# nmndeep/Robust-Segmentation

Hardware: AMD Instinct MI355X
Metric: SEA attack-iterations/sec (UperNet-CNX-T, 512x512) (higher is better)
Workload: dtype f32 (frozen-weight GEMMs on the 16-bit matrix cores by operand splitting: fp16x2 (22 significant bits per operand, 3 MFMA products) forward, fp16x2 (22 significant bits per operand, 3 MFMA products) input gradient; fp32 storage and accumulate)

## Files before the change

include/sea_hip.h:

```cpp
#ifndef SEA_HIP_H
#define SEA_HIP_H

#include <stddef.h>
#include <stdint.h>

#ifdef __cplusplus
extern "C" {
#endif

#define SEA_MODE_MASK_CE 0
#define SEA_MODE_MASK_CE_BAL 1
#define SEA_MODE_JS 2
#define SEA_MODE_CE 3

#define SEA_DTYPE_F32 0
#define SEA_DTYPE_BF16 1
#define SEA_DTYPE_F16 2

#define SEA_LAYOUT_NCHW 0
#define SEA_LAYOUT_NHWC 1

int sea_abi_version(void);
const char* sea_build_info(void);
int sea_fastdiv_magic(uint32_t d, uint32_t* m, uint32_t* s);
// ... 74 lines not shown
int sea_dwconv7x7_nhwc(const float* x, const float* wt, const float* bias, float* y, int B, int C,
                       int H, int W, int flip, void* stream);
int sea_dwconv7x7_nhwc_add(const float* x, const float* wt, const float* bias, const float* addend, float* y, int B,
                           int C, int H, int W, int flip, void* stream);

int sea_upsample_bilinear_fwd(const float* x, float* y, int64_t planes, int h, int w, int H, int W,
                              void* stream);
int sea_upsample_bilinear_bwd(const float* gy, float* gx, int64_t planes, int h, int w, int H, int W,
                              void* stream);
int sea_upsample_bilinear_nhwc_fwd(const float* x, const float* residual, float* y, int B, int C, int h,
                                   int w, int H, int W, int64_t y_pixel_stride, void* stream);
int sea_upsample_bilinear_nhwc_bwd(const float* gy, float* gx, int B, int C, int h, int w, int H, int W,
                                   int64_t gy_pixel_stride, void* stream);

int64_t sea_wino_tiles(int B, int H, int W, int m);
int sea_wino_input_transform(const float* x, int64_t x_pixel_stride, const float* gate, const float* scale,
                             float* V, int64_t v_tile_stride, int B, int C, int H, int W, int m, void* stream);
int sea_wino_filter_transform(const float* w, float* U, int Cout, int Cin, int m, int flip, void* stream);
int sea_wino_input_transform_amax(const float* x, int64_t x_pixel_stride, const float* gate, const float* scale, float* V,
                                  int64_t v_tile_stride, int B, int C, int H, int W, int m, uint32_t* amax_out, void* stream);
int sea_wino_output_transform(const float* M, const float* addend, const float* scale, const float* bias,
                              int relu, float* y, int B, int C, int H, int W, int m, void* stream);

int sea_layernorm_fwd(const float* x, const float* w, const float* b, float* y, float* mean, float* rstd,
                      int64_t rows, int C, float eps, void* stream);
int sea_layernorm_bwd(const float* g, const float* x, const float* w, const float* mean, const float* rstd,
                      float* dx, int64_t rows, int C, void* stream);

int64_t sea_dwconv7x7_nhwc_wgrad_workspace(int B, int C, int H);
int sea_dwconv7x7_nhwc_wgrad(const float* x, const float* gy, float* gw, float* gb, float* ws, int B, int C, int H, int W,
                             void* stream);

int sea_adaptive_avg_pool_nhwc_fwd(const float* x, float* out, int B, int C, int H, int W, int oh, int ow, void* stream);
int sea_adaptive_avg_pool_nhwc_bwd(const float* g, float* dx, int B, int C, int H, int W, int oh, int ow, void* stream);

int sea_stem_conv1_ln_gelu(const float* x, const float* w, const float* bias, const float* gamma, const float* beta,
                           float* y, float* a, int B, int CO, int H, int W, float eps, void* stream);
int sea_stem_conv1_bwd(const float* dy, const float* w, float* dx, int B, int CO, int H, int W, void* stream);
int sea_ln_gelu_cl_fwd(const float* y, const float* gamma, const float* beta, float* a, int a_nchw, int B, int C, int64_t HW,
                       float eps, void* stream);
int sea_ln_gelu_cl_bwd(const float* da, int a_nchw, const float* y, const float* gamma, const float* beta, float* dy, int B,
                       int C, int64_t HW, float eps, void* stream);

int sea_tap_gather_fwd(const float* G, float* extra, int accumulate, int B, int C, int h, int w, int H, int W,
                       void* stream);
int sea_tap_gather_bwd(const float* gz, float* dG, int B, int C, int h, int w, int H, int W, void* stream);
int sea_gate_scale(const float* g, const float* gate, const float* scale, float* out, int64_t pixels, int C,
                   void* stream);

int sea_nchw_to_nhwc(const float* in, const float* scale, float* out, int B, int C, int64_t HW, void* stream);
int sea_nhwc_to_nchw(const float* in, const float* scale, const float* residual, float* out, int B, int C,
                     int64_t HW, void* stream);

int sea_patch2x2(const float* src, float* dst, int B, int H, int W, int C, int inverse, void* stream);

int sea_attention_fwd(const float* q, const float* k, const float* v, int64_t sb, int64_t sh, int64_t st, int B, int H,
                      int T, int D, float scale, float* out, float* lse, void* stream);
int sea_attention_bwd(const float* q, const float* k, const float* v, int64_t sb, int64_t sh, int64_t st, int B, int H,
                      int T, int D, float scale, const float* out, const float* grad_out, const float* lse,
                      float* delta, float* dq, float* dk, float* dv, int64_t gsb, int64_t gsh, int64_t gst,
                      void* stream);
int sea_attention_bwd_terms(const float* q, const float* k, const float* v, int64_t sb, int64_t sh, int64_t st, int B, int H,
                            int T, int D, float scale, const float* out, const float* grad_out, const float* lse,
                            float* delta, float* dq, float* dk, float* dv, int64_t gsb, int64_t gsh, int64_t gst,
                            int terms, void* stream);
int sea_attention_fwd_terms(const float* q, const float* k, const float* v, int64_t sb, int64_t sh, int64_t st, int B, int H,
                            int T, int D, float scale, float* out, float* lse, int terms, void* stream);
int sea_attention_fwd_f16(const float* q, const float* k, const float* v, int64_t sb, int64_t sh, int64_t st, int B, int H,
                          int T, int D, float scale, uint32_t* amax_ws, float* out, float* lse, void* stream);
int sea_attention_bwd_f16(const float* q, const float* k, const float* v, int64_t sb, int64_t sh, int64_t st, int B, int H,
                          int T, int D, float scale, const float* out, const float* grad_out, const float* lse,
                          float* delta, uint32_t* amax_ws, float* dq, float* dk, float* dv, int64_t gsb, int64_t gsh,
                          int64_t gst, void* stream);

int64_t sea_gemm_split_packed_bytes(int N, int K, int terms);
int sea_absmax_bits(const float* A, int64_t lda, int M, int K, int batch, int64_t strideA, int rows_per_word,
                    uint32_t* out_bits, void* stream);
int sea_gemm_split_f16(const float* A, int64_t lda, const void* Wp, float* C, int64_t ldc, const float* bias, int relu, int M,
                       int N, int K, int batch, int64_t strideA, int64_t strideW_bytes, int64_t strideC,
                       const uint32_t* amax_bits, int amax_rows, uint32_t* out_amax, void* stream);
int sea_gemm_split_pack(const float* W, int64_t ldw, int trans, int N, int K, int terms, void* out, void* stream);
int sea_gemm_splitk_reduce(const float* partial, int splits, int M, int N, const float* bias, const float* addend,
                           int64_t ld_addend, int relu, float* C, int64_t ldc, uint32_t* out_amax, void* stream);
typedef struct SeaGemmEpilogue {
  const float* addend;
  int64_t ld_addend, stride_addend;
  float* gelu_out;
  const float* gelu_grad_of;
  const float* a_gelu_grad_of;
  int a_gate;
  int a_gelu;
  float a_amax_mul;
  const float* a_amax_mul_dev;
} SeaGemmEpilogue;
int sea_gemm_split_fused(const float* A, int64_t lda, const void* Wp, float* C, int64_t ldc, const float* bias, int relu, int M,
                         int N, int K, int terms, int batch, int64_t strideA, int64_t strideW_bytes, int64_t strideC,
                         const uint32_t* amax_bits, int amax_rows, uint32_t* out_amax, const SeaGemmEpilogue* epi,
                         void* stream);
int sea_gemm_split(const float* A, int64_t lda, const void* Wp, float* C, int64_t ldc, const float* bias, int relu, int M,
                   int N, int K, int terms, int batch, int64_t strideA, int64_t strideW_bytes, int64_t strideC,
                   void* stream);
int sea_classifier_supported(int P, int K, int cls);
int sea_classifier_fwd(const float* y, const float* W, const float* bias, float* out, int B, int P, int K, int cls, void* stream);
int sea_classifier_bwd(const float* g, const float* W, float* gy, int B, int P, int K, int cls, const float* gate,
                       const float* gate_scale, void* stream);
int sea_mlp_fused_supported(int C, int H);
int sea_ln_mlp_fused_fwd(const float* x, int64_t ldx, const float* ln_w, const float* ln_b, float ln_eps, const void* W1p,
                         const float* b1, const void* W2p, const float* b2, const float* res, int64_t ldres, float* y,
                         int64_t ldy, int M, int C, int H, const uint32_t* amax_x, const uint32_t* amax_h, void* stream);
int sea_ln_mlp_fused_bwd(const float* g, int64_t ldg, const float* x, int64_t ldx, const float* ln_w, const float* ln_b,
                         float ln_eps, const void* W1p, const float* b1, const void* W2tp, const void* W1tp, float* dx,
                         int64_t lddx, int M, int C, int H, const uint32_t* amax_x, const float* amax_mul_dev, void* stream);
int sea_probe_gelu_mismatches(unsigned long long* out, void* stream);
int sea_probe_ln_rows(const float* x, const float* ln_w, const float* ln_b, float eps, int M, int C, float* yn, float* mean,
                      float* rstd, void* stream);
int sea_mlp_fused_stamps(int bwd, const float* g, int64_t ldg, const float* x, int64_t ldx, const void* W1p, const float* b1,
                         const void* W2p, const void* W1tp, const float* b2, const float* res, float* y, int M, int C,
                         const uint32_t* amax_x, const uint32_t* amax_h, const float* amax_mul_dev, unsigned long long* dbg,
                         void* stream);
int sea_mlp_fused_fwd(const float* x, int64_t ldx, const void* W1p, const float* b1, const void* W2p, const float* b2,
                      const float* res, int64_t ldres, float* y, int64_t ldy, int M, int C, int H, const uint32_t* amax_x,
                      const uint32_t* amax_h, void* stream);
int sea_mlp_fused_bwd(const float* g, int64_t ldg, const float* x, int64_t ldx, const void* W1p, const float* b1,
                      const void* W2tp, const void* W1tp, float* dx, int64_t lddx, int M, int C, int H,
                      const uint32_t* amax_x, const float* amax_mul_dev, void* stream);
int sea_gemm_split_mfma_shape(int shape);
int sea_gemm_split_pipeline(int pipe);

int sea_probe_stream_copy(const void* src, void* dst, size_t bytes, int non_temporal, void* stream);
int sea_probe_stream_read(const void* src, float* sink, size_t bytes, void* stream);

#define SEA_MSF_MAX_CLASSES 192
int sea_msf_resize_input(const float* x, float* y, float* y_flip, int64_t planes, int h, int w, int H, int W,
                         void* stream);
int sea_msf_accumulate(const float* logits, float* score, int B, int C, int hl, int wl, int Hs, int Ws, int H, int W,
                       int flip, void* stream);

int sea_psp_polyphase_split(const float* x, float* y, int B, int H, int W, int C, int d, int first_only, void* stream);
int sea_psp_polyphase_merge(const float* y, float* x, int B, int H, int W, int C, int d, int first_only, void* stream);
int sea_psp_upsample_ac(const float* x, float* y, int64_t planes, int h, int w, int H, int W, void* stream);
int sea_psp_upsample_ac_bwd(const float* gy, float* gx, float* work, int64_t planes, int h, int w, int H, int W,
                            void* stream);
int sea_psp_upsample_ac_nhwc(const float* x, float* y, int B, int C, int h, int w, int H, int W, int S, void* stream);
int sea_psp_upsample_ac_nhwc_bwd(const float* gy, float* gx, float* work, int B, int C, int h, int w, int H, int W,
                                 int S, void* stream);
int sea_psp_add_relu(const float* a, const float* r, float* y, int64_t n, void* stream);
int sea_psp_add_relu_bwd(const float* gy, const float* y, float* gx, int64_t n, void* stream);

int64_t sea_bn_train_workspace_floats(int64_t M, int C);
int sea_bn_train_fwd(const float* x, const float* r, const float* gamma, const float* beta, float* y, float* mean,
                     float* invstd, float* scale, float* running_mean, float* running_var, int64_t* num_batches_tracked,
                     float* work, int64_t M, int C, float eps, float momentum, int relu, void* stream);
int sea_bn_train_bwd(const float* g, const float* x, const float* y, const float* mean, const float* invstd,
                     const float* scale, float* dx, float* dgamma, float* dbeta, float* gr, float* work, int64_t M, int C,
                     int relu, void* stream);

#ifdef __cplusplus
}
#endif
#endif
```

robust-segmentation_amd/csrc/gemm_split.h:

```cpp
#pragma once
#include "sea_common.h"
#include <atomic>

namespace sea {

typedef __bf16 bf16x8 __attribute__((ext_vector_type(8)));
typedef __bf16 bf16x2 __attribute__((ext_vector_type(2)));
typedef float f32x2 __attribute__((ext_vector_type(2)));
typedef float f32x16 __attribute__((ext_vector_type(16)));
typedef float f32x4 __attribute__((ext_vector_type(4)));
typedef uint32_t u32x4 __attribute__((ext_vector_type(4)));
typedef uint32_t u32x2 __attribute__((ext_vector_type(2)));
typedef _Float16 f16x8 __attribute__((ext_vector_type(8)));
typedef _Float16 f16x2 __attribute__((ext_vector_type(2)));

constexpr int GS_BM = 128, GS_BN = 128, GS_BK = 32;
constexpr int GS_IMG = GS_BM * GS_BK * 2;

__device__ __forceinline__ uint32_t pack_bf16(float a, float b) {
  const f32x2 v = {a, b};
  return __builtin_bit_cast(uint32_t, __builtin_convertvector(v, bf16x2));
}

template <int TERMS>
__device__ __forceinline__ void split4(const f32x4 v, u32x2 (&out)[TERMS]) {
  float r0 = v[0], r1 = v[1], r2 = v[2], r3 = v[3];
#pragma unroll
  for (int t = 0; t < TERMS; ++t) {
    const uint32_t p0 = pack_bf16(r0, r1), p1 = pack_bf16(r2, r3);
    out[t] = u32x2{p0, p1};
    if (t + 1 < TERMS) {
      r0 -= __uint_as_float(p0 << 16);
      r1 -= __uint_as_float(p0 & 0xffff0000u);
      r2 -= __uint_as_float(p1 << 16);
      r3 -= __uint_as_float(p1 & 0xffff0000u);
    }
  }
}

__device__ __forceinline__ uint32_t pack_f16(float a, float b) {
  const f32x2 v = {a, b};
  return __builtin_bit_cast(uint32_t, __builtin_convertvector(v, f16x2));
}
__device__ __forceinline__ void split4_f16(const f32x4 v, float s, u32x2 (&out)[2]) {
  const float a0 = v[0] * s, a1 = v[1] * s, a2 = v[2] * s, a3 = v[3] * s;
  const uint32_t h0 = pack_f16(a0, a1), h1 = pack_f16(a2, a3);
  const f32x2 f0 = __builtin_convertvector(__builtin_bit_cast(f16x2, h0), f32x2);
  const f32x2 f1 = __builtin_convertvector(__builtin_bit_cast(f16x2, h1), f32x2);
  out[0] = u32x2{h0, h1};
  out[1] = u32x2{pack_f16(a0 - f0[0], a1 - f0[1]), pack_f16(a2 - f1[0], a3 - f1[1])};
}
__device__ __host__ __forceinline__ void pow2_scale(uint32_t amax_bits, float& scale, float& inv) {
  int E = (int)((amax_bits >> 23) & 0xffu);
  E = E < 14 ? 14 : (E > 253 ? 253 : E);
  const uint32_t sb = (uint32_t)(267 - E) << 23, ib = (uint32_t)(E - 13) << 23;
  scale = __builtin_bit_cast(float, sb);
  inv = __builtin_bit_cast(float, ib);
}

template <bool S16>
__device__ __forceinline__ int swz(int row, int chunk) {
  return S16 ? ((chunk ^ ((0 - (row >> 2)) & 3)) << 4) : ((chunk ^ ((row >> 2) & 3)) << 4);
}
typedef float f32x4v __attribute__((ext_vector_type(4)));

struct GemmSplitArgs {
  const float* A;
  const char* W;
  float* C;
  const float* bias;
  int64_t lda, ldc, strideA, strideW, strideC;
  int M, N, K, Npad;
  int mblocks, nblocks, total, per_xcd;
  int relu;
  const uint32_t* amax_bits;
  int amax_rows;
  float amax_mul;
  const float* amax_mul_dev;
  const float* w_inv;
  uint32_t* out_amax;
  const float* addend;
  int64_t ld_add, stride_add;
  float* gelu_out;
  const float* gelu_grad_of;
  const float* a_gelu_grad_of;
  int a_gelu;
  int a_gate;
  int ko;
};

__device__ __forceinline__ float gelu_f(float x) { return 0.5f * x * (1.f + erff(x * 0.70710678118654752440f)); }
__device__ __forceinline__ float gelu_grad_f(float x) {
  const float cdf = 0.5f * (1.f + erff(x * 0.70710678118654752440f));
  const float pdf = __expf(-0.5f * x * x) * 0.39894228040143267794f;
  return cdf + x * pdf;
}

template <bool F16, bool EPI, int KO = 0>
__device__ __forceinline__ void gemm_split_store_tile(const GemmSplitArgs& p, const f32x16 (&acc)[2][2], int g, int m0, int n0,
                                                      char* smem, const float* row_inv, const float (&bv_c)[2],
                                                      const float (&wi_c)[2]) {
  const int M = p.M, N = p.N;
  const int64_t ldc = p.ldc, ld_add = p.ld_add;
  const int relu = p.relu;
  const int lane = threadIdx.x & 63, wave = threadIdx.x >> 6;
  const int wn = wave & 1, r = lane & 31, h = lane >> 5;
  const float* const addg = (EPI && p.addend) ? p.addend + (int64_t)g * p.stride_add : nullptr;
  float* const gelu_out = (EPI && p.gelu_out) ? p.gelu_out + (int64_t)g * p.strideC : nullptr;
  const float* const gelu_src = (EPI && p.gelu_grad_of) ? p.gelu_grad_of + (int64_t)g * p.strideC : nullptr;
  const int wave_u = __builtin_amdgcn_readfirstlane(wave);
  const int row0_u = m0 + (wave_u >> 1) * 64;
  float* const Cg = p.C + (int64_t)g * p.strideC;
  char* const scr = smem + wave_u * 8192;
  const int lr = lane >> 4, lc = lane & 15;
  const int col4 = n0 + wn * 64 + 4 * lc;
  const bool vec = (((ldc | p.strideC | N) & 3) == 0) && ((((uintptr_t)p.C) & 15) == 0) &&
                   (!(EPI && addg) || ((((ld_add | p.stride_add) & 3) == 0) && ((((uintptr_t)p.addend) & 15) == 0))) &&
                   (!(EPI && gelu_out) || ((((uintptr_t)p.gelu_out) & 15) == 0)) &&
                   (!(EPI && gelu_src) || ((((uintptr_t)p.gelu_grad_of) & 15) == 0));
  const int off_c = lr * (int)ldc + col4;
  const int off_a = (EPI && addg) ? lr * (int)ld_add + col4 : 0;
  uint32_t omax = 0;
#pragma unroll
  for (int mi = 0; mi < 2; ++mi) {
    if (mi) asm volatile("s_waitcnt lgkmcnt(0)" ::: "memory");
#pragma unroll
    for (int ni = 0; ni < 2; ++ni) {
      const int col = n0 + wn * 64 + ni * 32 + r;
#pragma unroll
      for (int e = 0; e < 16; ++e) {
        const int row_l = (e & 3) + 8 * (e >> 2) + 4 * h;
        const float v = (F16 ? acc[mi][ni][e] * (row_inv[(wave_u >> 1) * 64 + mi * 32 + row_l] * wi_c[ni]) : acc[mi][ni][e]) + bv_c[ni];
        *(float*)(scr + row_l * 256 + (ni * 32 + r) * 4) = v;
      }
      (void)col;
    }
    asm volatile("s_waitcnt lgkmcnt(0)" ::: "memory");
#pragma unroll
    for (int k = 0; k < 8; ++k) {
      const int row_u = row0_u + mi * 32 + 4 * k;
      f32x4 v = *(const f32x4*)(scr + k * 1024 + lr * 256 + lc * 16);
      if (row_u + lr >= M || col4 >= N) continue;
      float* const crow = Cg + (int64_t)row_u * ldc;
      if (vec) {
        if (EPI && addg) v += *(const f32x4*)((addg + (int64_t)row_u * ld_add) + off_a);
        if (relu) {
#pragma unroll
          for (int e = 0; e < 4; ++e) v[e] = v[e] > 0.f ? v[e] : 0.f;
        }
        if (EPI && gelu_src) {
          const f32x4 t = *(const f32x4*)((gelu_src + (int64_t)row_u * ldc) + off_c);
#pragma unroll
          for (int e = 0; e < 4; ++e) v[e] *= gelu_grad_f(t[e]);
        }
        if constexpr ((KO & 64) != 0)
          __builtin_nontemporal_store(v, (f32x4*)(crow + off_c));
        else if ((KO & 1) == 0 || __float_as_uint(v[0]) == 0x7fc12345u)
          *(f32x4*)(crow + off_c) = v;
        if (EPI && gelu_out) {
          f32x4 o;
#pragma unroll
          for (int e = 0; e < 4; ++e) o[e] = gelu_f(v[e]);
          *(f32x4*)((gelu_out + (int64_t)row_u * ldc) + off_c) = o;
        }
#pragma unroll
        for (int e = 0; e < 4; ++e) {
          const uint32_t vb = __float_as_uint(v[e]) & 0x7fffffffu;
          omax = vb > omax ? vb : omax;
        }
      } else {
#pragma unroll
        for (int e = 0; e < 4; ++e) {
          if (col4 + e < N) {
            float x = v[e];
            if (EPI && addg) x += (addg + (int64_t)row_u * ld_add)[off_a + e];
            if (relu) x = x > 0.f ? x : 0.f;
            if (EPI && gelu_src) x *= gelu_grad_f((gelu_src + (int64_t)row_u * ldc)[off_c + e]);
            crow[off_c + e] = x;
            if (EPI && gelu_out) (gelu_out + (int64_t)row_u * ldc)[off_c + e] = gelu_f(x);
            const uint32_t vb = __float_as_uint(x) & 0x7fffffffu;
            omax = vb > omax ? vb : omax;
          }
        }
      }
    }
  }
  if (p.out_amax != nullptr) {
#pragma unroll
    for (int o = 32; o > 0; o >>= 1) {
      const uint32_t other = (uint32_t)__shfl_xor((int)omax, o, 64);
      omax = other > omax ? other : omax;
    }
    if (lane == 0 && omax > *(volatile uint32_t*)p.out_amax) atomicMax(p.out_amax, omax);
  }
}

bool gemm_split_pp_launch(const GemmSplitArgs& p, int terms, int pro, bool fused, hipStream_t st);
bool gemm_split_big_launch(GemmSplitArgs p, int terms, int batch, int shape, int pro, hipStream_t st);

}
```

robust-segmentation_amd/csrc/gemm_split.hip:

```cpp
#include "gemm_split.h"

namespace sea {

template <int TERMS, bool S16, bool F16 = false, bool EPI = false, int PRO = 0>
__global__ __launch_bounds__(256, 3) void gemm_split_kernel(const GemmSplitArgs p) {
  __shared__ __attribute__((aligned(16))) char smem[2 * TERMS * GS_IMG < 32768 ? 32768 : 2 * TERMS * GS_IMG];
  char* As = smem;
  char* Bs = smem + TERMS * GS_IMG;

  const int M = p.M, N = p.N, K = p.K, Npad = p.Npad;
  const int64_t lda = p.lda, ldc = p.ldc;
  const int logical = (int)(blockIdx.x & 7) * p.per_xcd + (int)(blockIdx.x >> 3);
  if ((int)(blockIdx.x >> 3) >= p.per_xcd || logical >= p.total) return;
  const int nb = logical % p.nblocks;
  const int t2 = logical / p.nblocks;
  const int mb = t2 % p.mblocks;
  const int g = t2 / p.mblocks;
  const int m0 = mb * GS_BM, n0 = nb * GS_BN;
  const float* const w_inv = F16 ? (const float*)((const char*)p.w_inv + (int64_t)g * p.strideW) : nullptr;

  const int tid = threadIdx.x, lane = tid & 63, wave = tid >> 6;
  const int wm = wave >> 1, wn = wave & 1;
  const int r = lane & 31, h = lane >> 5;

  const int q = tid & 7, arow = tid >> 3;
  const char* const Abase = (const char*)(p.A + (int64_t)g * p.strideA);
  float* const Cbase = p.C;
  const float* const bias = p.bias;
  const int64_t strideC = p.strideC;
  const int relu = p.relu;
  const float* const addg = (EPI && p.addend) ? p.addend + (int64_t)g * p.stride_add : nullptr;
  const int64_t ld_add = p.ld_add;
  float* const gelu_out = (EPI && p.gelu_out) ? p.gelu_out + (int64_t)g * p.strideC : nullptr;
  const float* const gelu_src = (EPI && p.gelu_grad_of) ? p.gelu_grad_of + (int64_t)g * p.strideC : nullptr;
  __shared__ float row_sc[F16 ? GS_BM : 1], row_inv[F16 ? GS_BM : 1];
  float a_sc[4] = {1.f, 1.f, 1.f, 1.f};
  auto load_row_scales = [&]() {
   if constexpr (F16) {
    if (tid < GS_BM) {
      int row = m0 + tid;
      row = row < M ? row : M - 1;
      float sc, inv;
      uint32_t word = p.amax_bits[p.amax_rows > 0 ? row / p.amax_rows : 0];
      const float mul = p.amax_mul_dev ? *p.amax_mul_dev : p.amax_mul;
      if (mul != 1.f) word = __float_as_uint(__uint_as_float(word) * mul) & 0x7fffffffu;
      pow2_scale(word, sc, inv);
      row_sc[tid] = sc;
      row_inv[tid] = inv;
    }
    __syncthreads();
#pragma unroll
    for (int i = 0; i < 4; ++i) a_sc[i] = row_sc[arow + 32 * i];
   }
  };
  uint32_t aoff[4];
#pragma unroll
  for (int i = 0; i < 4; ++i) {
    int row = m0 + arow + 32 * i;
    row = row < M ? row : M - 1;
    aoff[i] = (uint32_t)(((int64_t)row * lda + 4 * q) * 4);
  }
  const char* const Wbase = p.W + (int64_t)g * p.strideW + (int64_t)n0 * 64;
  const int64_t w_term = (int64_t)Npad * 64, w_kb = (int64_t)TERMS * w_term;
  const uint32_t woff = (uint32_t)tid * 16;

  f32x4 pa[4];
  f32x4 pt[(PRO == 1 || PRO == 3) ? 4 : 1];
  const char* const Tbase = (PRO == 1 || PRO == 3) ? (const char*)(p.a_gelu_grad_of + (int64_t)g * p.strideA) : nullptr;
  u32x4 pw[2 * TERMS];
  auto fetch = [&](int kb) {
    const char* a = Abase + (int64_t)kb * (GS_BK * 4);
#pragma unroll
    for (int i = 0; i < 4; ++i) pa[i] = *(const f32x4*)(a + aoff[i]);
    if constexpr (PRO == 1 || PRO == 3) {
      const char* t = Tbase + (int64_t)kb * (GS_BK * 4);
#pragma unroll
      for (int i = 0; i < 4; ++i) pt[i] = *(const f32x4*)(t + aoff[i]);
    }
    const char* w = Wbase + (int64_t)kb * w_kb;
#pragma unroll
    for (int i = 0; i < 2 * TERMS; ++i) pw[i] = *(const u32x4*)(w + (int64_t)(i >> 1) * w_term + (i & 1) * 4096 + woff);
  };
  auto stage = [&]() {
#pragma unroll
    for (int i = 0; i < 4; ++i) {
      u32x2 s[TERMS];
      if constexpr (PRO == 1) {
#pragma unroll
        for (int e = 0; e < 4; ++e) pa[i][e] *= gelu_grad_f(pt[i][e]);
      }
      if constexpr (PRO == 2) {
#pragma unroll
        for (int e = 0; e < 4; ++e) pa[i][e] = gelu_f(pa[i][e]);
      }
      if constexpr (PRO == 3) {
#pragma unroll
        for (int e = 0; e < 4; ++e) pa[i][e] = pt[i][e] > 0.f ? pa[i][e] : 0.f;
      }
      if constexpr (F16)
        split4_f16(pa[i], a_sc[i], s);
      else
        split4<TERMS>(pa[i], s);
      const int row = arow + 32 * i;
#pragma unroll
      for (int t = 0; t < TERMS; ++t) *(u32x2*)(As + t * GS_IMG + row * 64 + swz<S16>(row, q >> 1) + (q & 1) * 8) = s[t];
    }
#pragma unroll
    for (int i = 0; i < 2 * TERMS; ++i) {
      const int pc = tid + 256 * i, term = pc >> 9, row = (pc & 511) >> 2, chunk = pc & 3;
      *(u32x4*)(Bs + term * GS_IMG + row * 64 + swz<S16>(row, chunk)) = pw[i];
    }
  };

  const int nkb = K / GS_BK;
  float* Cg = Cbase + (int64_t)g * strideC;
  if constexpr (!S16) {
    f32x16 acc[2][2];
#pragma unroll
    for (int mi = 0; mi < 2; ++mi)
#pragma unroll
      for (int ni = 0; ni < 2; ++ni)
#pragma unroll
        for (int e = 0; e < 16; ++e) acc[mi][ni][e] = 0.f;
    fetch(0);
    load_row_scales();
    float bv_c[2], wi_c[2];
#pragma unroll
    for (int ni = 0; ni < 2; ++ni) {
      const int col = n0 + wn * 64 + ni * 32 + r;
      bv_c[ni] = (bias && col < N) ? bias[col] : 0.f;
      wi_c[ni] = (F16 && col < N) ? w_inv[col] : 1.f;
    }
    for (int kb = 0; kb < nkb; ++kb) {
      stage();
      __syncthreads();
      fetch(kb + 1 < nkb ? kb + 1 : kb);
      __builtin_amdgcn_sched_barrier(0);
#pragma unroll
      for (int s = 0; s < 2; ++s) {
        bf16x8 a[2][TERMS], b[2][TERMS];
#pragma unroll
        for (int mi = 0; mi < 2; ++mi) {
          const int row = wm * 64 + mi * 32 + r;
#pragma unroll
          for (int t = 0; t < TERMS; ++t)
            a[mi][t] = *(const bf16x8*)(As + t * GS_IMG + row * 64 + swz<false>(row, 2 * s + h));
        }
#pragma unroll
        for (int ni = 0; ni < 2; ++ni) {
          const int row = wn * 64 + ni * 32 + r;
#pragma unroll
          for (int t = 0; t < TERMS; ++t)
            b[ni][t] = *(const bf16x8*)(Bs + t * GS_IMG + row * 64 + swz<false>(row, 2 * s + h));
        }
#pragma unroll
        for (int mi = 0; mi < 2; ++mi)
#pragma unroll
          for (int ni = 0; ni < 2; ++ni) {
            f32x16 c = acc[mi][ni];
            if constexpr (F16) {
              c = __builtin_amdgcn_mfma_f32_32x32x16_f16(__builtin_bit_cast(f16x8, a[mi][1]), __builtin_bit_cast(f16x8, b[ni][0]), c, 0, 0, 0);
              c = __builtin_amdgcn_mfma_f32_32x32x16_f16(__builtin_bit_cast(f16x8, a[mi][0]), __builtin_bit_cast(f16x8, b[ni][1]), c, 0, 0, 0);
              c = __builtin_amdgcn_mfma_f32_32x32x16_f16(__builtin_bit_cast(f16x8, a[mi][0]), __builtin_bit_cast(f16x8, b[ni][0]), c, 0, 0, 0);
            } else {
              if constexpr (TERMS == 3) {
                c = __builtin_amdgcn_mfma_f32_32x32x16_bf16(a[mi][2], b[ni][0], c, 0, 0, 0);
                c = __builtin_amdgcn_mfma_f32_32x32x16_bf16(a[mi][0], b[ni][2], c, 0, 0, 0);
                c = __builtin_amdgcn_mfma_f32_32x32x16_bf16(a[mi][1], b[ni][1], c, 0, 0, 0);
              }
              if constexpr (TERMS >= 2) {
                c = __builtin_amdgcn_mfma_f32_32x32x16_bf16(a[mi][1], b[ni][0], c, 0, 0, 0);
                c = __builtin_amdgcn_mfma_f32_32x32x16_bf16(a[mi][0], b[ni][1], c, 0, 0, 0);
              }
              c = __builtin_amdgcn_mfma_f32_32x32x16_bf16(a[mi][0], b[ni][0], c, 0, 0, 0);
            }
            acc[mi][ni] = c;
          }
      }
      __syncthreads();
    }
    gemm_split_store_tile<F16, EPI>(p, acc, g, m0, n0, smem, row_inv, bv_c, wi_c);
  } else {
    const int r16 = lane & 15, c16 = lane >> 4;
    f32x4v acc[4][4];
#pragma unroll
    for (int mi = 0; mi < 4; ++mi)
#pragma unroll
      for (int ni = 0; ni < 4; ++ni) acc[mi][ni] = f32x4v{0.f, 0.f, 0.f, 0.f};
    fetch(0);
    load_row_scales();
    for (int kb = 0; kb < nkb; ++kb) {
      stage();
      __syncthreads();
      fetch(kb + 1 < nkb ? kb + 1 : kb);
      __builtin_amdgcn_sched_barrier(0);
#pragma unroll
      for (int nh = 0; nh < 2; ++nh) {
        bf16x8 b[2][TERMS];
#pragma unroll
        for (int nj = 0; nj < 2; ++nj) {
          const int row = wn * 64 + (2 * nh + nj) * 16 + r16;
#pragma unroll
          for (int t = 0; t < TERMS; ++t) b[nj][t] = *(const bf16x8*)(Bs + t * GS_IMG + row * 64 + swz<true>(row, c16));
        }
#pragma unroll
        for (int mi = 0; mi < 4; ++mi) {
          bf16x8 a[TERMS];
          const int row = wm * 64 + mi * 16 + r16;
#pragma unroll
          for (int t = 0; t < TERMS; ++t) a[t] = *(const bf16x8*)(As + t * GS_IMG + row * 64 + swz<true>(row, c16));
#pragma unroll
          for (int nj = 0; nj < 2; ++nj) {
            f32x4v c = acc[mi][2 * nh + nj];
            if constexpr (F16) {
              c = __builtin_amdgcn_mfma_f32_16x16x32_f16(__builtin_bit_cast(f16x8, a[1]), __builtin_bit_cast(f16x8, b[nj][0]), c, 0, 0, 0);
              c = __builtin_amdgcn_mfma_f32_16x16x32_f16(__builtin_bit_cast(f16x8, a[0]), __builtin_bit_cast(f16x8, b[nj][1]), c, 0, 0, 0);
              c = __builtin_amdgcn_mfma_f32_16x16x32_f16(__builtin_bit_cast(f16x8, a[0]), __builtin_bit_cast(f16x8, b[nj][0]), c, 0, 0, 0);
            } else {
              if constexpr (TERMS == 3) {
                c = __builtin_amdgcn_mfma_f32_16x16x32_bf16(a[2], b[nj][0], c, 0, 0, 0);
                c = __builtin_amdgcn_mfma_f32_16x16x32_bf16(a[0], b[nj][2], c, 0, 0, 0);
                c = __builtin_amdgcn_mfma_f32_16x16x32_bf16(a[1], b[nj][1], c, 0, 0, 0);
              }
              if constexpr (TERMS >= 2) {
                c = __builtin_amdgcn_mfma_f32_16x16x32_bf16(a[1], b[nj][0], c, 0, 0, 0);
                c = __builtin_amdgcn_mfma_f32_16x16x32_bf16(a[0], b[nj][1], c, 0, 0, 0);
              }
              c = __builtin_amdgcn_mfma_f32_16x16x32_bf16(a[0], b[nj][0], c, 0, 0, 0);
            }
            acc[mi][2 * nh + nj] = c;
          }
          __builtin_amdgcn_sched_barrier(0);
        }
      }
      __syncthreads();
    }
    uint32_t omax16 = 0;
#pragma unroll
    for (int ni = 0; ni < 4; ++ni) {
      const int col = n0 + wn * 64 + ni * 16 + r16;
      if (col >= N) continue;
      const float bv = bias ? bias[col] : 0.f;
      const float wi = F16 ? w_inv[col] : 1.f;
#pragma unroll
      for (int mi = 0; mi < 4; ++mi) {
#pragma unroll
        for (int e = 0; e < 4; ++e) {
          const int row = m0 + wm * 64 + mi * 16 + 4 * c16 + e;
          if (row < M) {
            float v = (F16 ? acc[mi][ni][e] * (row_inv[row - m0] * wi) : acc[mi][ni][e]) + bv;
            if (EPI && addg) v += addg[(int64_t)row * ld_add + col];
            if (relu) v = v > 0.f ? v : 0.f;
            if (EPI && gelu_src) v *= gelu_grad_f(gelu_src[(int64_t)row * ldc + col]);
            Cg[(int64_t)row * ldc + col] = v;
            if (EPI && gelu_out) gelu_out[(int64_t)row * ldc + col] = gelu_f(v);
            const uint32_t vb = __float_as_uint(v) & 0x7fffffffu;
            omax16 = vb > omax16 ? vb : omax16;
          }
        }
      }
    }
    if (p.out_amax != nullptr) {
#pragma unroll
      for (int o = 32; o > 0; o >>= 1) {
        const uint32_t other = (uint32_t)__shfl_xor((int)omax16, o, 64);
        omax16 = other > omax16 ? other : omax16;
      }
      if (lane == 0 && omax16 > *(volatile uint32_t*)p.out_amax) atomicMax(p.out_amax, omax16);
    }
  }
}

template <int TERMS>
__global__ void gemm_split_pack_kernel(const float* __restrict__ W, int64_t ldw, int trans, int N, int K, int Npad,
                                       uint16_t* __restrict__ out) {
  const int64_t total = (int64_t)(K / 32) * Npad * 32;
  for (int64_t i = (int64_t)blockIdx.x * blockDim.x + threadIdx.x; i < total; i += (int64_t)gridDim.x * blockDim.x) {
    const int kk = (int)(i & 31);
    const int64_t t = i >> 5;
    const int n = (int)(t % Npad);
    const int kb = (int)(t / Npad);
    const int k = kb * 32 + kk;
    float rem = 0.f;
    if (n < N) rem = trans ? W[(int64_t)k * ldw + n] : W[(int64_t)n * ldw + k];
#pragma unroll
    for (int term = 0; term < TERMS; ++term) {
      const uint32_t pk = pack_bf16(rem, 0.f);
      out[(((int64_t)kb * TERMS + term) * Npad + n) * 32 + kk] = (uint16_t)(pk & 0xffffu);
      rem -= __uint_as_float(pk << 16);
    }
  }
}

__global__ __launch_bounds__(256) void absmax_bits_kernel(const float* __restrict__ A, int64_t lda, int M, int K4,
                                                          int64_t strideA, int batch, uint32_t* __restrict__ out) {
  uint32_t m = 0;
  auto take = [&](const f32x4 v) {
#pragma unroll
    for (int e = 0; e < 4; ++e) {
      const uint32_t b = __float_as_uint(v[e]) & 0x7fffffffu;
      m = b > m ? b : m;
    }
  };
  if (lda == (int64_t)4 * K4 && (batch == 1 || strideA == (int64_t)M * lda)) {
    const int64_t total = (int64_t)batch * M * K4, stride = (int64_t)gridDim.x * blockDim.x;
    const f32x4* p = reinterpret_cast<const f32x4*>(A);
    for (int64_t i = (int64_t)blockIdx.x * blockDim.x + threadIdx.x; i < total; i += 2 * stride) {
      const int64_t j = i + stride;
      const f32x4 v0 = p[i], v1 = p[j < total ? j : i];
      take(v0);
      take(v1);
    }
  } else {
    const int64_t rows = (int64_t)batch * M;
    for (int64_t r = blockIdx.x; r < rows; r += gridDim.x) {
      const int64_t g = r / M;
      const float* row = A + g * strideA + (r - g * M) * lda;
      for (int k4 = threadIdx.x; k4 < K4; k4 += blockDim.x) take(*reinterpret_cast<const f32x4*>(row + 4 * k4));
    }
  }
#pragma unroll
  for (int o = 32; o > 0; o >>= 1) {
    const uint32_t other = (uint32_t)__shfl_xor((int)m, o, 64);
    m = other > m ? other : m;
  }
  __shared__ uint32_t wave_max[4];
  if ((threadIdx.x & 63) == 0) wave_max[threadIdx.x >> 6] = m;
  __syncthreads();
  if (threadIdx.x == 0) {
    uint32_t b = wave_max[0];
#pragma unroll
    for (int w = 1; w < 4; ++w) b = wave_max[w] > b ? wave_max[w] : b;
    if (b) atomicMax(out, b);
  }
}

__global__ void rowmax_bits_kernel(const float* __restrict__ W, int64_t ldw, int trans, int N, int K, uint32_t* __restrict__ out) {
  const int n = blockIdx.x;
  uint32_t m = 0;
  for (int k = threadIdx.x; k < K; k += blockDim.x) {
    const uint32_t b = __float_as_uint(trans ? W[(int64_t)k * ldw + n] : W[(int64_t)n * ldw + k]) & 0x7fffffffu;
    m = b > m ? b : m;
  }
#pragma unroll
  for (int o = 32; o > 0; o >>= 1) {
    const uint32_t other = (uint32_t)__shfl_xor((int)m, o, 64);
    m = other > m ? other : m;
  }
  if ((threadIdx.x & 63) == 0 && m) atomicMax(out + n, m);
}

__global__ void gemm_split_pack_f16_kernel(const float* __restrict__ W, int64_t ldw, int trans, int N, int K, int Npad,
// ... 124 lines not shown
    }
  }
  if (out_amax != nullptr) {
#pragma unroll
    for (int o = 32; o > 0; o >>= 1) {
      const uint32_t other = (uint32_t)__shfl_xor((int)omax, o, 64);
      omax = other > omax ? other : omax;
    }
    if ((threadIdx.x & 63) == 0 && omax > *(volatile uint32_t*)out_amax) atomicMax(out_amax, omax);
  }
}

}

using namespace sea;

static inline int gs_npad(int N) { return (N + GS_BN - 1) / GS_BN * GS_BN; }

static std::atomic<int> g_mfma_shape{[] {
  const char* e = getenv("SEA_GEMM_SHAPE");
  return (e && e[0] == '1') ? 16 : 32;
}()};

static const int g_wide_min = [] {
  const char* e = getenv("SEA_GEMM_WIDE_MIN");
  return e ? atoi(e) : 192;
}();

static std::atomic<int> g_pipeline{[] {
  const char* e = getenv("SEA_GEMM_PIPE");
  return (e && e[0] >= '0' && e[0] <= '3') ? e[0] - '0' : 2;
}()};

extern "C" int sea_gemm_split_pipeline(int pipe) {
  const int prev = g_pipeline.load(std::memory_order_relaxed);
  if (pipe >= 0 && pipe <= 3) g_pipeline.store(pipe, std::memory_order_relaxed);
  return prev;
}

extern "C" int sea_gemm_split_mfma_shape(int shape) {
  const int prev = g_mfma_shape.load(std::memory_order_relaxed);
  if (shape == 16 || shape == 32) g_mfma_shape.store(shape, std::memory_order_relaxed);
  return prev;
}

extern "C" int64_t sea_gemm_split_packed_bytes(int N, int K, int terms) {
  if (N <= 0 || K <= 0 || K % GS_BK || (terms != 1 && terms != 2 && terms != 3 && terms != 22)) return -1;
  if (terms == 22) return (int64_t)(K / GS_BK) * 2 * gs_npad(N) * GS_BK * 2 + (int64_t)gs_npad(N) * 8;
  return (int64_t)(K / GS_BK) * terms * gs_npad(N) * GS_BK * 2;
}

extern "C" int sea_gemm_split_pack(const float* W, int64_t ldw, int trans, int N, int K, int terms, void* out,
                                   void* stream) {
  SEA_CHECK_ARG(W && out && N > 0 && K > 0 && (K % GS_BK) == 0 && (terms == 1 || terms == 2 || terms == 3 || terms == 22));
  SEA_CHECK_ARG(ldw >= (trans ? N : K));
  const int Npad = gs_npad(N);
  const int64_t total = (int64_t)(K / 32) * Npad * 32;
  const int grid = grid_for(total, 256);
  if (terms == 22) {
    char* base = (char*)out;
    float* w_inv = (float*)(base + (int64_t)(K / GS_BK) * 2 * Npad * GS_BK * 2);
    uint32_t* rowmax = (uint32_t*)(w_inv + Npad);
    hipLaunchKernelGGL(zero_words_kernel, dim3((Npad + 255) / 256), dim3(256), 0, (hipStream_t)stream, rowmax, Npad);
    hipLaunchKernelGGL(rowmax_bits_kernel, dim3(N), dim3(256), 0, (hipStream_t)stream, W, ldw, trans, N, K, rowmax);
    hipLaunchKernelGGL(gemm_split_pack_f16_kernel, dim3(grid), dim3(256), 0, (hipStream_t)stream, W, ldw, trans, N, K, Npad,
                       rowmax, (uint16_t*)out, w_inv);
    SEA_RETURN_LAST();
  }
  if (terms == 1)
    hipLaunchKernelGGL(gemm_split_pack_kernel<1>, dim3(grid), dim3(256), 0, (hipStream_t)stream, W, ldw, trans, N, K, Npad,
                       (uint16_t*)out);
  else if (terms == 3)
    hipLaunchKernelGGL(gemm_split_pack_kernel<3>, dim3(grid), dim3(256), 0, (hipStream_t)stream, W, ldw, trans, N, K, Npad,
                       (uint16_t*)out);
  else
    hipLaunchKernelGGL(gemm_split_pack_kernel<2>, dim3(grid), dim3(256), 0, (hipStream_t)stream, W, ldw, trans, N, K, Npad,
                       (uint16_t*)out);
  SEA_RETURN_LAST();
}

static int gemm_split_impl(const float* A, int64_t lda, const void* Wp, float* C, int64_t ldc, const float* bias, int relu, int M,
                           int N, int K, int terms, int batch, int64_t strideA, int64_t strideW_bytes, int64_t strideC,
                           const uint32_t* amax_bits, int amax_rows, uint32_t* out_amax, void* stream,
                           const SeaGemmEpilogue* epi = nullptr);

extern "C" int sea_gemm_split(const float* A, int64_t lda, const void* Wp, float* C, int64_t ldc, const float* bias,
                              int relu, int M, int N, int K, int terms, int batch, int64_t strideA, int64_t strideW_bytes,
                              int64_t strideC, void* stream) {
  SEA_CHECK_ARG(terms == 1 || terms == 2 || terms == 3);
  return gemm_split_impl(A, lda, Wp, C, ldc, bias, relu, M, N, K, terms, batch, strideA, strideW_bytes, strideC, nullptr, 0,
                         nullptr, stream);
}

extern "C" int sea_gemm_split_f16(const float* A, int64_t lda, const void* Wp, float* C, int64_t ldc, const float* bias,
                                  int relu, int M, int N, int K, int batch, int64_t strideA, int64_t strideW_bytes,
                                  int64_t strideC, const uint32_t* amax_bits, int amax_rows, uint32_t* out_amax,
                                  void* stream) {
  SEA_CHECK_ARG(amax_bits != nullptr && amax_rows >= 0);
  return gemm_split_impl(A, lda, Wp, C, ldc, bias, relu, M, N, K, 22, batch, strideA, strideW_bytes, strideC, amax_bits,
                         amax_rows, out_amax, stream);
}

extern "C" int sea_gemm_split_fused(const float* A, int64_t lda, const void* Wp, float* C, int64_t ldc, const float* bias,
                                    int relu, int M, int N, int K, int terms, int batch, int64_t strideA,
                                    int64_t strideW_bytes, int64_t strideC, const uint32_t* amax_bits, int amax_rows,
                                    uint32_t* out_amax, const SeaGemmEpilogue* epi, void* stream) {
  SEA_CHECK_ARG(terms == 1 || terms == 2 || terms == 3 || (terms == 22 && amax_bits != nullptr && amax_rows >= 0));
  SEA_CHECK_ARG(terms == 22 || out_amax == nullptr);
  if (epi) {
    SEA_CHECK_ARG(!epi->addend || epi->ld_addend >= N);
    SEA_CHECK_ARG(!(epi->gelu_out && epi->gelu_grad_of) && !(relu && (epi->gelu_out || epi->gelu_grad_of)));
    SEA_CHECK_ARG(!(epi->a_gelu_grad_of || epi->a_gelu) || !(epi->addend || epi->gelu_out || epi->gelu_grad_of));
    SEA_CHECK_ARG(!(epi->a_gelu_grad_of && epi->a_gelu));
  }
  return gemm_split_impl(A, lda, Wp, C, ldc, bias, relu, M, N, K, terms, batch, strideA, strideW_bytes, strideC,
                         terms == 22 ? amax_bits : nullptr, amax_rows, out_amax, stream, epi);
}

extern "C" int sea_gemm_splitk_reduce(const float* partial, int splits, int M, int N, const float* bias, const float* addend,
                                      int64_t ld_addend, int relu, float* C, int64_t ldc, uint32_t* out_amax, void* stream) {
  SEA_CHECK_ARG(partial && C && splits >= 1 && M > 0 && N > 0 && (N % 4) == 0 && ldc >= N && (ldc % 4) == 0);
  SEA_CHECK_ARG(((((uintptr_t)partial) | ((uintptr_t)C) | ((uintptr_t)bias) | ((uintptr_t)addend)) & 15) == 0);
  SEA_CHECK_ARG(!addend || (ld_addend >= N && (ld_addend % 4) == 0));
  const int64_t total = (int64_t)M * (N / 4);
  hipLaunchKernelGGL(splitk_reduce_kernel, dim3(grid_for(total, 256)), dim3(256), 0, (hipStream_t)stream, (const f32x4*)partial,
                     splits, total, M, N / 4, (const f32x4*)bias, relu, C, ldc, out_amax, addend, ld_addend);
  SEA_RETURN_LAST();
}

extern "C" int sea_absmax_bits(const float* A, int64_t lda, int M, int K, int batch, int64_t strideA, int rows_per_word,
                               uint32_t* out_bits, void* stream) {
  SEA_CHECK_ARG(A && out_bits && M > 0 && K > 0 && (K % 4) == 0 && (lda % 4) == 0 && batch > 0 && (((uintptr_t)A) & 15) == 0);
  SEA_CHECK_ARG(rows_per_word >= 0);
  if (rows_per_word == 1 && batch == 1) {
    const int K4 = K / 4;
    const int lpr = K4 >= 64 ? 64 : (K4 >= 32 ? 32 : (K4 >= 16 ? 16 : 8));
    const int64_t blocks = ((int64_t)M * lpr + 255) / 256;
    const dim3 grid((unsigned)(blocks < 8192 ? blocks : 8192)), block(256);
    if (lpr == 64)
      hipLaunchKernelGGL(rowmax_rows_kernel<64>, grid, block, 0, (hipStream_t)stream, A, lda, M, K4, out_bits);
    else if (lpr == 32)
      hipLaunchKernelGGL(rowmax_rows_kernel<32>, grid, block, 0, (hipStream_t)stream, A, lda, M, K4, out_bits);
    else if (lpr == 16)
      hipLaunchKernelGGL(rowmax_rows_kernel<16>, grid, block, 0, (hipStream_t)stream, A, lda, M, K4, out_bits);
    else
      hipLaunchKernelGGL(rowmax_rows_kernel<8>, grid, block, 0, (hipStream_t)stream, A, lda, M, K4, out_bits);
    SEA_RETURN_LAST();
  }
  if (rows_per_word > 0 && rows_per_word < M) {
    const int words = (M + rows_per_word - 1) / rows_per_word;
    SEA_CHECK_ARG(words <= 65535);
    hipLaunchKernelGGL(zero_words_kernel, dim3((words + 255) / 256), dim3(256), 0, (hipStream_t)stream, out_bits, words);
    const int64_t per = (int64_t)rows_per_word * (K / 4);
    int gx = (int)((per + 1023) / 1024);
    gx = gx < 1 ? 1 : (gx > 64 ? 64 : gx);
    hipLaunchKernelGGL(absmax_groups_kernel, dim3(gx, words), dim3(256), 0, (hipStream_t)stream, A, lda, M, K / 4, strideA, batch,
                       rows_per_word, out_bits);
    SEA_RETURN_LAST();
  }
  hipLaunchKernelGGL(zero_words_kernel, dim3(1), dim3(64), 0, (hipStream_t)stream, out_bits, 1);
  const int64_t total = (int64_t)batch * M * (K / 4);
  int grid = grid_for(total, 512);
  if (grid > 1024) grid = 1024;
  hipLaunchKernelGGL(absmax_bits_kernel, dim3(grid), dim3(256), 0, (hipStream_t)stream, A, lda, M, K / 4, strideA, batch, out_bits);
  SEA_RETURN_LAST();
}

static int gemm_split_impl(const float* A, int64_t lda, const void* Wp, float* C, int64_t ldc, const float* bias, int relu, int M,
                           int N, int K, int terms, int batch, int64_t strideA, int64_t strideW_bytes, int64_t strideC,
                           const uint32_t* amax_bits, int amax_rows, uint32_t* out_amax, void* stream,
                           const SeaGemmEpilogue* epi) {
  SEA_CHECK_ARG(A && Wp && C && M > 0 && N > 0 && K > 0 && (K % GS_BK) == 0 && batch > 0);
  SEA_CHECK_ARG(lda >= K && ldc >= N && (lda % 4) == 0 && (int64_t)M * lda < (1ll << 30));
  SEA_CHECK_ARG(((((uintptr_t)A) | ((uintptr_t)Wp)) & 15) == 0 && (((uintptr_t)C) & 3) == 0 && (strideA % 4) == 0 &&
                (strideW_bytes % 16) == 0);
  GemmSplitArgs p = {};
  p.A = A;
  p.W = (const char*)Wp;
  p.C = C;
  p.bias = bias;
  p.lda = lda;
  p.ldc = ldc;
  p.strideA = strideA;
  p.strideW = strideW_bytes;
  p.strideC = strideC;
  p.M = M;
  p.N = N;
  p.K = K;
  p.Npad = gs_npad(N);
  p.mblocks = (M + GS_BM - 1) / GS_BM;
  p.nblocks = p.Npad / GS_BN;
  const int64_t total = (int64_t)p.mblocks * p.nblocks * batch;
  SEA_CHECK_ARG(total < (1ll << 30));
  p.total = (int)total;
  p.per_xcd = (p.total + 7) / 8;
  p.relu = relu;
  p.amax_bits = amax_bits;
  p.amax_rows = amax_rows;
  p.out_amax = out_amax;
  p.addend = epi ? epi->addend : nullptr;
  p.ld_add = epi ? epi->ld_addend : 0;
  p.stride_add = epi ? epi->stride_addend : 0;
  p.gelu_out = epi ? epi->gelu_out : nullptr;
  p.gelu_grad_of = epi ? epi->gelu_grad_of : nullptr;
  p.a_gelu_grad_of = epi ? epi->a_gelu_grad_of : nullptr;
  p.a_gelu = epi ? epi->a_gelu : 0;
  p.a_gate = epi ? epi->a_gate : 0;
  p.amax_mul = (epi && epi->a_amax_mul > 0.f) ? epi->a_amax_mul : 1.f;
  p.amax_mul_dev = epi ? epi->a_amax_mul_dev : nullptr;
  p.w_inv = terms == 22 ? (const float*)((const char*)Wp + (int64_t)(K / GS_BK) * 2 * gs_npad(N) * GS_BK * 2) : nullptr;
  const dim3 grid(p.per_xcd * 8), block(256);
  const bool shape16 = g_mfma_shape.load(std::memory_order_relaxed) == 16;
  const bool fused = p.addend || p.gelu_out || p.gelu_grad_of;
  SEA_CHECK_ARG(!(p.a_gelu && (fused || p.a_gelu_grad_of)) && (!p.a_gelu_grad_of || !fused));
  SEA_CHECK_ARG(!p.a_gelu_grad_of || ((terms == 1 || terms == 2 || terms == 22) && (((uintptr_t)p.a_gelu_grad_of) & 15) == 0));
  const int pro = p.a_gelu ? 2 : (p.a_gelu_grad_of ? (p.a_gate ? 3 : 1) : 0);
  const hipStream_t st = (hipStream_t)stream;
  const int pipe = g_pipeline.load(std::memory_order_relaxed);
  if (!shape16 && (terms == 22 || terms == 2) && !fused && (pipe == 2 || pipe == 3)) {
    const int64_t t256 = (N % 256) == 0 ? (int64_t)((M + 255) / 256) * (N / 256) * batch : 0;
    const int64_t t384 = (N % 384) == 0 ? (int64_t)((M + 127) / 128) * (N / 384) * batch : 0;
    if (pro == 0 && M >= 256 && t256 > 0 && (pipe == 3 ? t384 == 0 : t256 >= 1024) && gemm_split_big_launch(p, terms, batch, 0, 0, st))
      SEA_RETURN_LAST();
    const bool wide_fits = t384 >= g_wide_min && t384 <= 256 && K >= 192;
    if (t384 > 0 && M >= 128 && (pipe == 3 || wide_fits) && gemm_split_big_launch(p, terms, batch, 1, pro, st)) SEA_RETURN_LAST();
  }
  const int64_t r2 = (total + 511) / 512 * 512, r3 = (total + 767) / 768 * 768;
  const bool pingpong = pipe == 1 || (pipe == 2 && pro != 0 && r2 <= r3);
  if (!shape16 && terms != 3 && pingpong && gemm_split_pp_launch(p, terms, pro, fused, st)) SEA_RETURN_LAST();
#define SEA_GS_LAUNCH(T, S16, F16, EPI, PRO) hipLaunchKernelGGL((gemm_split_kernel<T, S16, F16, EPI, PRO>), grid, block, 0, st, p)
#define SEA_GS_PRO(T, S16, F16)                                   \
  do {                                                            \
    if (pro == 2) SEA_GS_LAUNCH(T, S16, F16, false, 2);           \
    else if (pro == 1) SEA_GS_LAUNCH(T, S16, F16, false, 1);      \
    else if (pro == 3) SEA_GS_LAUNCH(T, S16, F16, false, 3);      \
    else if (fused) SEA_GS_LAUNCH(T, S16, F16, true, 0);          \
    else SEA_GS_LAUNCH(T, S16, F16, false, 0);                    \
  } while (0)
  if (terms == 22) {
    if (shape16) SEA_GS_PRO(2, true, true); else SEA_GS_PRO(2, false, true);
  } else if (terms == 3) {
    SEA_CHECK_ARG(pro == 0 || pro == 2);
    if (shape16) {
      if (pro == 2) SEA_GS_LAUNCH(3, true, false, false, 2); else if (fused) SEA_GS_LAUNCH(3, true, false, true, 0); else SEA_GS_LAUNCH(3, true, false, false, 0);
    } else {
      if (pro == 2) SEA_GS_LAUNCH(3, false, false, false, 2); else if (fused) SEA_GS_LAUNCH(3, false, false, true, 0); else SEA_GS_LAUNCH(3, false, false, false, 0);
    }
  } else if (terms == 1) {
    if (shape16) SEA_GS_PRO(1, true, false); else SEA_GS_PRO(1, false, false);
  } else {
    if (shape16) SEA_GS_PRO(2, true, false); else SEA_GS_PRO(2, false, false);
  }
#undef SEA_GS_PRO
#undef SEA_GS_LAUNCH
  SEA_RETURN_LAST();
}
```

robust-segmentation_amd/csrc/gemm_split_big.hip:

```cpp
#include "gemm_split.h"

namespace sea {

template <bool F16, int WM, int WN, int TN, int PRO, int DEPTH, int MI = 2, bool WDMA = false>
__global__ __launch_bounds__(64 * WM * WN) void gemm_split_big_kernel(const GemmSplitArgs p) {
  static_assert(WM * WN == 8 || (WM * WN == 4 && MI == 4), "eight waves, or four with 128-row wave tiles");
  constexpr int TERMS = 2;
  constexpr int NT = 64 * WM * WN;
  constexpr int RP = NT / 8;
  constexpr int BM = 32 * MI * WM, WT = 32 * TN, BN = WT * WN;
  constexpr int IMG_A = BM * 64, IMG_W = BN * 64;
  constexpr int STAGE = TERMS * (IMG_A + IMG_W);
  constexpr int NA = BM / RP;
  constexpr int NWT = BN * 4 / NT, NW = TERMS * NWT;
  constexpr int SLOTS = 3 * MI * TN;
  constexpr int UNIT_EVERY = SLOTS / (3 * NA);
  constexpr bool HAS_T = (PRO == 1 || PRO == 3);
  static_assert(STAGE == 65536 && SLOTS % (3 * NA) == 0 && NW + 2 <= SLOTS, "configuration");
  constexpr int NBLK = TERMS * BN / 16;
  constexpr int NVM = NA * (HAS_T ? 2 : 1);
  static_assert(!WDMA || (NT == 512 && NBLK % 8 == 0 && DEPTH == 1), "LDS-DMA weights: eight waves, one register set");
  extern __shared__ __attribute__((aligned(16))) char smem[];
  float* const row_sc = (float*)(smem + 2 * STAGE);
  float* const row_inv = row_sc + BM;

  const int M = p.M, N = p.N, K = p.K, Npad = p.Npad;
  const int64_t lda = p.lda, ldc = p.ldc;
  const int logical = (int)(blockIdx.x & 7) * p.per_xcd + (int)(blockIdx.x >> 3);
  if ((int)(blockIdx.x >> 3) >= p.per_xcd || logical >= p.total) return;
  const int nb = logical % p.nblocks;
  const int t2 = logical / p.nblocks;
  const int mb = t2 % p.mblocks;
  const int g = t2 / p.mblocks;
  const int m0 = mb * BM, n0 = nb * BN;
  const float* const w_inv = F16 ? (const float*)((const char*)p.w_inv + (int64_t)g * p.strideW) : nullptr;

  const int tid = threadIdx.x, lane = tid & 63, wave = tid >> 6;
  const int wm = wave / WN, wn = wave % WN;
  const int r = lane & 31, h = lane >> 5;
  const int q = tid & 7, arow = tid >> 3;

  const char* const Abase = (const char*)(p.A + (int64_t)g * p.strideA);
  const char* const Tbase = HAS_T ? (const char*)(p.a_gelu_grad_of + (int64_t)g * p.strideA) : nullptr;
  const float* const bias = p.bias;
  const int nkb = K / GS_BK;
  const char* const Wbase = p.W + (int64_t)g * p.strideW + (int64_t)n0 * 64;
  const int64_t w_term = (int64_t)Npad * 64, w_kb = (int64_t)TERMS * w_term;
  const uint32_t woff = (uint32_t)tid * 16;
  const uint32_t a_bytes = (uint32_t)((((int64_t)(M - 1)) * lda + K) * 4);
  const uint32_t w_bytes = (uint32_t)((int64_t)nkb * w_kb - (int64_t)n0 * 64);

  float a_sc[NA];
#pragma unroll
  for (int i = 0; i < NA; ++i) a_sc[i] = 1.f;
  const uint32_t aoff0 = (uint32_t)(((int64_t)(m0 + arow) * lda + 4 * q) * 4);
  const uint32_t a_wr0 = (uint32_t)(arow * 64 + swz<false>(arow, q >> 1) + (q & 1) * 8);
  const int wrow0 = tid >> 2;
  const uint32_t w_wr0 = (uint32_t)(TERMS * IMG_A + wrow0 * 64 + swz<false>(wrow0, tid & 3));
  const int a_row_step = (int)(RP * lda * 4);
  const int ra = wm * 32 * MI + r, rb = wn * WT + r;
  const uint32_t a_rd = (uint32_t)(ra * 64 + swz<false>(ra, h));
  const uint32_t b_rd = (uint32_t)(TERMS * IMG_A + rb * 64 + swz<false>(rb, h));

  struct Tile {
    f32x4 a[NA];
    f32x4 t[HAS_T ? NA : 1];
    u32x4 w[WDMA ? 1 : NW];
  };
  Tile R0 = {}, R1 = {};
  auto fetch_a = [&](Tile& R, int kb) __attribute__((always_inline)) {
    f32x4 (&Ra)[NA] = R.a;
    f32x4 (&Rt)[HAS_T ? NA : 1] = R.t;
    const int live = kb < nkb ? (int)a_bytes : 0;
    const __amdgpu_buffer_rsrc_t rs = __builtin_amdgcn_make_buffer_rsrc((void*)Abase, 0, live, 0x00020000);
#pragma unroll
    for (int i = 0; i < NA; ++i)
      Ra[i] = __builtin_bit_cast(f32x4, __builtin_amdgcn_raw_buffer_load_b128(
          rs, (int)((m0 + arow + RP * i < M) ? aoff0 : a_bytes), kb * (GS_BK * 4) + i * a_row_step, 0));
    if constexpr (HAS_T) {
      const __amdgpu_buffer_rsrc_t rt = __builtin_amdgcn_make_buffer_rsrc((void*)Tbase, 0, live, 0x00020000);
#pragma unroll
      for (int i = 0; i < NA; ++i)
        Rt[i] = __builtin_bit_cast(f32x4, __builtin_amdgcn_raw_buffer_load_b128(
            rt, (int)((m0 + arow + RP * i < M) ? aoff0 : a_bytes), kb * (GS_BK * 4) + i * a_row_step, 0));
    }
  };
  const int wave_u0 = __builtin_amdgcn_readfirstlane(wave);
  const uint32_t lane_off = (uint32_t)((lane >> 2) * 64 + (((lane & 3) ^ ((lane >> 4) & 3)) * 16));
  auto dma_w = [&](char* stage, int kb) __attribute__((always_inline)) {
    if constexpr (WDMA) {
      const int kbc = kb < nkb ? kb : nkb - 1;
#pragma unroll
      for (int i = 0; i < NBLK / 8; ++i) {
        const int blk = wave_u0 + 8 * i;
        const int t = blk / (BN / 16), rb16 = blk - t * (BN / 16);
        const char* const src = Wbase + (int64_t)kbc * w_kb + (int64_t)t * w_term + rb16 * 1024 + lane_off;
        __builtin_amdgcn_global_load_lds((const __attribute__((address_space(1))) void*)src,
                                         (__attribute__((address_space(3))) void*)(stage + TERMS * IMG_A + blk * 1024), 16, 0, 0);
      }
    }
  };
  auto fetch_w = [&](Tile& R, int kb) __attribute__((always_inline)) {
    if constexpr (WDMA) return;
    u32x4 (&Rw)[WDMA ? 1 : NW] = R.w;
    const __amdgpu_buffer_rsrc_t rs = __builtin_amdgcn_make_buffer_rsrc((void*)Wbase, 0, kb < nkb ? (int)w_bytes : 0, 0x00020000);
#pragma unroll
    for (int i = 0; i < NW; ++i)
      Rw[i] = __builtin_bit_cast(u32x4, __builtin_amdgcn_raw_buffer_load_b128(
                                            rs, (int)woff, kb * (int)w_kb + (i / NWT) * (int)w_term + (i % NWT) * (16 * NT), 0));
  };
  auto write_w = [&](Tile& R, int i, char* stage) __attribute__((always_inline)) {
    if constexpr (!WDMA) *(u32x4*)(stage + w_wr0 + (i / NWT) * IMG_W + (i % NWT) * (16 * NT)) = R.w[i];
  };

  f32x4 sv;
  uint32_t hi_a, hi_b;
  auto unit_a = [&](Tile& R, int i, int part, char* stage) __attribute__((always_inline)) {
    f32x4 (&Rt)[HAS_T ? NA : 1] = R.t;
    if (part == 0) {
      f32x4 v = R.a[i];
      if constexpr (PRO == 1) {
#pragma unroll
        for (int e = 0; e < 4; ++e) v[e] *= gelu_grad_f(Rt[i][e]);
      }
      if constexpr (PRO == 2) {
#pragma unroll
// ... 145 lines not shown
    unit_a(R0, i, 1, st0);
    unit_a(R0, i, 2, st0);
  }
#pragma unroll
  for (int i = 0; i < NW; ++i) write_w(R0, i, st0);
  fetch_a(R0, DEPTH);
  fetch_w(R0, DEPTH);
  if constexpr (WDMA) asm volatile("s_waitcnt vmcnt(%0)" ::"n"(NVM) : "memory");
  __syncthreads();
  read_a(st0, 0);
#pragma unroll
  for (int ni = 0; ni < TN; ++ni) read_b(st0, 0, ni);
  int kb = 0;
  for (; kb + 2 <= nkb; kb += 2) {
    step(st0, st1, RB, kb + 1 + DEPTH);
    step(st1, st0, RA, kb + 2 + DEPTH);
  }
  if (kb < nkb) step(st0, st1, RB, nkb);
#undef SEA_PIN

  float bv_c[TN], wi_c[TN];
#pragma unroll
  for (int ni = 0; ni < TN; ++ni) {
    const int col = n0 + wn * WT + ni * 32 + r;
    bv_c[ni] = (bias && col < N) ? bias[col] : 0.f;
    wi_c[ni] = (F16 && col < N) ? w_inv[col] : 1.f;
  }
  const int wave_u = __builtin_amdgcn_readfirstlane(wave);
  const int row0_u = m0 + (wave_u / WN) * 32 * MI;
  float* const Cg = p.C + (int64_t)g * p.strideC;
  constexpr int SCR = 32 * WT * 4;
  char* const scr = smem + wave_u * SCR;
  constexpr int F4_ROW = WT / 4;
  const bool vec = (((ldc | p.strideC | N) & 3) == 0) && ((((uintptr_t)p.C) & 15) == 0);
  const int relu = p.relu;
  uint32_t omax = 0;
#pragma unroll
  for (int mi = 0; mi < MI; ++mi) {
    if (mi) asm volatile("s_waitcnt lgkmcnt(0)" ::: "memory");
#pragma unroll
    for (int ni = 0; ni < TN; ++ni) {
#pragma unroll
      for (int e = 0; e < 16; ++e) {
        const int row_l = (e & 3) + 8 * (e >> 2) + 4 * h;
        const float v = (F16 ? acc[mi][ni][e] * (row_inv[(wave_u / WN) * 32 * MI + mi * 32 + row_l] * wi_c[ni]) : acc[mi][ni][e]) + bv_c[ni];
        *(float*)(scr + (row_l * WT + ni * 32 + r) * 4) = v;
      }
    }
    asm volatile("s_waitcnt lgkmcnt(0)" ::: "memory");
#pragma unroll
    for (int k = 0; k < WT / 8; ++k) {
      const int f = k * 64 + lane;
      const int row_l = f / F4_ROW, c4 = f - row_l * F4_ROW;
      f32x4 v = *(const f32x4*)(scr + f * 16);
      const int row = row0_u + mi * 32 + row_l, col4 = n0 + wn * WT + 4 * c4;
      if (row >= M || col4 >= N) continue;
      float* const cp = Cg + (int64_t)row * ldc + col4;
      if (relu) {
#pragma unroll
        for (int e = 0; e < 4; ++e) v[e] = v[e] > 0.f ? v[e] : 0.f;
      }
      if (vec) {
        *(f32x4*)cp = v;
      } else {
#pragma unroll
        for (int e = 0; e < 4; ++e)
          if (col4 + e < N) cp[e] = v[e];
      }
#pragma unroll
      for (int e = 0; e < 4; ++e) {
        const uint32_t vb = (col4 + e < N) ? (__float_as_uint(v[e]) & 0x7fffffffu) : 0u;
        omax = vb > omax ? vb : omax;
      }
    }
  }
  if (p.out_amax != nullptr) {
#pragma unroll
    for (int o = 32; o > 0; o >>= 1) {
      const uint32_t other = (uint32_t)__shfl_xor((int)omax, o, 64);
      omax = other > omax ? other : omax;
    }
    if (lane == 0 && omax > *(volatile uint32_t*)p.out_amax) atomicMax(p.out_amax, omax);
  }
}

template <bool F16, int WM, int WN, int TN, int PRO, int DEPTH, int MI = 2, bool WDMA = false>
static void big_launch_one(const GemmSplitArgs& p, hipStream_t st) {
  constexpr int lds = 2 * 65536 + 2 * 32 * MI * WM * (int)sizeof(float);
  auto k = gemm_split_big_kernel<F16, WM, WN, TN, PRO, DEPTH, MI, WDMA>;
  static bool attr_set_dev[64] = {};
  int dev = 0;
  (void)hipGetDevice(&dev);
  if (!attr_set_dev[dev & 63]) {
    (void)hipFuncSetAttribute((const void*)k, hipFuncAttributeMaxDynamicSharedMemorySize, lds);
    attr_set_dev[dev & 63] = true;
  }
  hipLaunchKernelGGL(k, dim3(p.per_xcd * 8), dim3(64 * WM * WN), (size_t)lds, st, p);
}

bool gemm_split_big_launch(GemmSplitArgs p, int terms, int batch, int shape, int pro, hipStream_t st) {
  const int BM = shape ? 128 : 256, BN = shape ? 384 : 256;
  if (p.ldc >= (1ll << 28) || p.lda >= (1ll << 22) || (p.N % BN) != 0 || p.Npad < p.N || (p.Npad % 128) != 0 || (shape == 0 && pro != 0))
    return false;
  if (p.Npad % BN) return false;
  p.mblocks = (p.M + BM - 1) / BM;
  p.nblocks = p.N / BN;
  const int64_t total = (int64_t)p.mblocks * p.nblocks * batch;
  if (total >= (1ll << 30)) return false;
  p.total = (int)total;
  p.per_xcd = (p.total + 7) / 8;
  const bool f16 = terms == 22;
  if (shape == 0) {
    const char* e = getenv("SEA_GEMM_BIG_WAVES");
    if (f16 && e && e[0] == '4') {
      big_launch_one<true, 2, 2, 4, 0, 1, 4>(p, st);
      return true;
    }
    const char* d = getenv("SEA_GEMM_WDMA");
    if (f16 && d && d[0] == '1') {
      big_launch_one<true, 4, 2, 4, 0, 1, 2, true>(p, st);
      return true;
    }
    if (f16) big_launch_one<true, 4, 2, 4, 0, 1>(p, st); else big_launch_one<false, 4, 2, 4, 0, 1>(p, st);
    return true;
  }
#define SEA_BIG_WIDE(F)                                              \
  do {                                                               \
    if (pro == 0) big_launch_one<F, 2, 4, 3, 0, 2>(p, st);           \
    else if (pro == 1) big_launch_one<F, 2, 4, 3, 1, 1>(p, st);      \
    else if (pro == 2) big_launch_one<F, 2, 4, 3, 2, 2>(p, st);      \
    else big_launch_one<F, 2, 4, 3, 3, 1>(p, st);                    \
  } while (0)
  if (f16) SEA_BIG_WIDE(true); else SEA_BIG_WIDE(false);
#undef SEA_BIG_WIDE
  return true;
}

}
```

robust-segmentation_amd/csrc/gemm_split_pp.hip:

```cpp
#include "gemm_split.h"

namespace sea {

template <int TERMS, bool F16, int KO = 0>
__device__ __forceinline__ void mfma_one(f32x16& c, const bf16x8 (&a)[TERMS], const bf16x8 (&b)[TERMS], int j) {
  constexpr int NP = TERMS == 2 ? 3 : 1;
  const int ia = (NP == 3 && j == 0) ? 1 : 0, ib = (NP == 3 && j == 1) ? 1 : 0;
  if constexpr ((KO & 8) != 0) {
    asm volatile("" ::"v"(a[ia]), "v"(b[ib]));
    return;
  }
  if constexpr (F16)
    c = __builtin_amdgcn_mfma_f32_32x32x16_f16(__builtin_bit_cast(f16x8, a[ia]), __builtin_bit_cast(f16x8, b[ib]), c, 0, 0, 0);
  else
    c = __builtin_amdgcn_mfma_f32_32x32x16_bf16(a[ia], b[ib], c, 0, 0, 0);
}

template <int TERMS, bool F16, bool EPI, int PRO, int DEPTH, int KO = 0>
__global__ __launch_bounds__(256, 2) void gemm_split_pp_kernel(const GemmSplitArgs p) {
  static_assert(TERMS == 1 || TERMS == 2, "ping-pong pipeline: one or two terms");
  constexpr int NP = TERMS == 2 ? 3 : 1;
  constexpr int STAGE = 2 * TERMS * GS_IMG;
  constexpr bool HAS_T = (PRO == 1 || PRO == 3);
  extern __shared__ __attribute__((aligned(16))) char smem[];
  float* const row_sc = (float*)(smem + 2 * STAGE);
  float* const row_inv = row_sc + GS_BM;

  const int M = p.M, N = p.N, K = p.K, Npad = p.Npad;
  const int64_t lda = p.lda, ldc = p.ldc;
  const int logical = (int)(blockIdx.x & 7) * p.per_xcd + (int)(blockIdx.x >> 3);
  if ((int)(blockIdx.x >> 3) >= p.per_xcd || logical >= p.total) return;
  const int nb = logical % p.nblocks;
  const int t2 = logical / p.nblocks;
  const int mb = t2 % p.mblocks;
  const int g = t2 / p.mblocks;
  const int m0 = mb * GS_BM, n0 = nb * GS_BN;
  const float* const w_inv = F16 ? (const float*)((const char*)p.w_inv + (int64_t)g * p.strideW) : nullptr;

  const int tid = threadIdx.x, lane = tid & 63, wave = tid >> 6;
  const int wm = wave >> 1, wn = wave & 1;
  const int r = lane & 31, h = lane >> 5;
  const int q = tid & 7, arow = tid >> 3;

  const char* const Abase = (const char*)(p.A + (int64_t)g * p.strideA);
  const char* const Tbase = HAS_T ? (const char*)(p.a_gelu_grad_of + (int64_t)g * p.strideA) : nullptr;
  const float* const bias = p.bias;
  const int relu = p.relu;
  const float* const addg = (EPI && p.addend) ? p.addend + (int64_t)g * p.stride_add : nullptr;
  const int64_t ld_add = p.ld_add;
  float* const gelu_out = (EPI && p.gelu_out) ? p.gelu_out + (int64_t)g * p.strideC : nullptr;
  const float* const gelu_src = (EPI && p.gelu_grad_of) ? p.gelu_grad_of + (int64_t)g * p.strideC : nullptr;

  float a_sc[4] = {1.f, 1.f, 1.f, 1.f};
  uint32_t aoff[4];
#pragma unroll
  for (int i = 0; i < 4; ++i) {
    int row = m0 + arow + 32 * i;
    row = row < M ? row : M - 1;
    aoff[i] = (uint32_t)(((int64_t)row * lda + 4 * q) * 4);
  }
  const char* const Wbase = p.W + (int64_t)g * p.strideW + (int64_t)n0 * 64;
  const int64_t w_term = (int64_t)Npad * 64, w_kb = (int64_t)TERMS * w_term;
  const uint32_t woff = (uint32_t)tid * 16;
  const int nkb = K / GS_BK;

  uint32_t a_wr[4];
#pragma unroll
  for (int i = 0; i < 4; ++i) {
    const int row = arow + 32 * i;
    a_wr[i] = (uint32_t)(row * 64 + swz<false>(row, q >> 1) + (q & 1) * 8);
  }
  uint32_t w_wr[2 * TERMS];
#pragma unroll
  for (int i = 0; i < 2 * TERMS; ++i) {
    const int pc = tid + 256 * i, term = pc >> 9, row = (pc & 511) >> 2, chunk = pc & 3;
    w_wr[i] = (uint32_t)(TERMS * GS_IMG + term * GS_IMG + row * 64 + swz<false>(row, chunk));
  }
  const int ra = wm * 64 + r, rb = wn * 64 + r;
  const uint32_t a_rd = (uint32_t)(ra * 64 + swz<false>(ra, h));
  const uint32_t b_rd = (uint32_t)(TERMS * GS_IMG + rb * 64 + swz<false>(rb, h));

  struct Tile {
    f32x4 a[4];
    f32x4 t[HAS_T ? 4 : 1];
    u32x4 w[2 * TERMS];
  };
  Tile R0 = {}, R1 = {};

  const uint32_t a_bytes = (KO && (p.ko & 2)) ? 0u : (uint32_t)((((int64_t)(M - 1)) * lda + K) * 4);
  const uint32_t w_bytes = (KO && (p.ko & 4)) ? 0u : (uint32_t)((int64_t)nkb * w_kb - (int64_t)n0 * 64);
  auto fetch_a = [&](Tile& R, int kb) __attribute__((always_inline)) {
    const int live = kb < nkb;
    const int soff = kb * (GS_BK * 4);
    const __amdgpu_buffer_rsrc_t ra_ = __builtin_amdgcn_make_buffer_rsrc((void*)Abase, 0, live ? (int)a_bytes : 0, 0x00020000);
#pragma unroll
    for (int i = 0; i < 4; ++i) R.a[i] = __builtin_bit_cast(f32x4, __builtin_amdgcn_raw_buffer_load_b128(ra_, (int)aoff[i], soff, 0));
    if constexpr (HAS_T) {
      const __amdgpu_buffer_rsrc_t rt_ = __builtin_amdgcn_make_buffer_rsrc((void*)Tbase, 0, live ? (int)a_bytes : 0, 0x00020000);
#pragma unroll
      for (int i = 0; i < 4; ++i) R.t[i] = __builtin_bit_cast(f32x4, __builtin_amdgcn_raw_buffer_load_b128(rt_, (int)aoff[i], soff, 0));
    }
  };
  auto fetch_w = [&](Tile& R, int kb) __attribute__((always_inline)) {
    const int live = kb < nkb;
    const __amdgpu_buffer_rsrc_t rw_ = __builtin_amdgcn_make_buffer_rsrc((void*)Wbase, 0, live ? (int)w_bytes : 0, 0x00020000);
#pragma unroll
    for (int i = 0; i < 2 * TERMS; ++i)
      R.w[i] = __builtin_bit_cast(u32x4, __builtin_amdgcn_raw_buffer_load_b128(
                                             rw_, (int)woff, kb * (int)w_kb + (i >> 1) * (int)w_term + (i & 1) * 4096, 0));
  };

  f32x4 sv;
  uint32_t hi_a, hi_b;
  auto unit_a = [&](Tile& R, int i, int part, char* stage) __attribute__((always_inline)) {
    if constexpr ((KO & 128) != 0) {
      if (part == 2) {
        *(u32x2*)(stage + a_wr[i]) = u32x2{__float_as_uint(R.a[i][0]), __float_as_uint(R.a[i][1])};
        if constexpr (TERMS == 2) *(u32x2*)(stage + GS_IMG + a_wr[i]) = u32x2{__float_as_uint(R.a[i][2]), __float_as_uint(R.a[i][3])};
      }
      return;
    }
    if (part == 0) {
      f32x4 v = R.a[i];
      if constexpr (PRO == 1) {
#pragma unroll
        for (int e = 0; e < 4; ++e) v[e] *= gelu_grad_f(R.t[i][e]);
      }
      if constexpr (PRO == 2) {
// ... 95 lines not shown
      for (int j = 0; j < NP; ++j) {
        mfma_one<TERMS, F16, KO>(acc[0][c], Ya[0], Yb[c], j);
        const int u = c * NP + j;
        if constexpr (NP == 3) {
          if (u < 2 * TERMS) unit_w(Rn, u < 2 * TERMS ? u : 0, nxt);
          if (u == 4) fetch_a(Rn, kf);
          if (u == 5) fetch_w(Rn, kf);
        } else {
          unit_w(Rn, u, nxt);
          if (u == 0) fetch_a(Rn, kf);
          if (u == 1) fetch_w(Rn, kf);
        }
        SEA_PIN();
      }
    }
    __syncthreads();
    read_frags(nxt, 0, Xa, Xb);
    SEA_PIN();
#pragma unroll
    for (int c = 0; c < 2; ++c) {
#pragma unroll
      for (int j = 0; j < NP; ++j) {
        mfma_one<TERMS, F16, KO>(acc[1][c], Ya[1], Yb[c], j);
        SEA_PIN();
      }
    }
  };

  char* const st0 = smem;
  char* const st1 = smem + STAGE;
  Tile& RA = R0;
  Tile& RB = DEPTH == 2 ? R1 : R0;
  fetch_a(R0, 0);
  fetch_w(R0, 0);
  if constexpr (DEPTH == 2) {
    fetch_a(R1, 1);
    fetch_w(R1, 1);
  }
  float bv_c[2], wi_c[2];
#pragma unroll
  for (int ni = 0; ni < 2; ++ni) {
    const int col = n0 + wn * 64 + ni * 32 + r;
    bv_c[ni] = (bias && col < N) ? bias[col] : 0.f;
    wi_c[ni] = (F16 && col < N) ? w_inv[col] : 1.f;
  }
  if constexpr (F16) {
    if (tid < GS_BM) {
      int row = m0 + tid;
      row = row < M ? row : M - 1;
      float sc, inv;
      uint32_t word = p.amax_bits[p.amax_rows > 0 ? row / p.amax_rows : 0];
      const float mul = p.amax_mul_dev ? *p.amax_mul_dev : p.amax_mul;
      if (mul != 1.f) word = __float_as_uint(__uint_as_float(word) * mul) & 0x7fffffffu;
      pow2_scale(word, sc, inv);
      row_sc[tid] = sc;
      row_inv[tid] = inv;
    }
    __syncthreads();
#pragma unroll
    for (int i = 0; i < 4; ++i) a_sc[i] = row_sc[arow + 32 * i];
  }
  SEA_PIN();
#pragma unroll
  for (int i = 0; i < 4; ++i) {
    unit_a(R0, i, 0, st0);
    unit_a(R0, i, 1, st0);
    unit_a(R0, i, 2, st0);
  }
#pragma unroll
  for (int i = 0; i < 2 * TERMS; ++i) unit_w(R0, i, st0);
  fetch_a(R0, DEPTH);
  fetch_w(R0, DEPTH);
  __syncthreads();
  read_frags(st0, 0, Xa, Xb);
  int kb = 0;
  for (; kb + 2 <= nkb; kb += 2) {
    step(st0, st1, RB, kb + 1 + DEPTH);
    step(st1, st0, RA, kb + 2 + DEPTH);
  }
  if (kb < nkb) step(st0, st1, RB, nkb);
#undef SEA_PIN

  gemm_split_store_tile<F16, EPI, KO>(p, acc, g, m0, n0, smem, row_inv, bv_c, wi_c);
}

template <int TERMS, bool F16, bool EPI, int PRO, int DEPTH>
static void pp_launch_one(const GemmSplitArgs& p, hipStream_t st) {
  constexpr int lds = 2 * 2 * TERMS * GS_IMG + (F16 ? 2 * GS_BM * (int)sizeof(float) : 0);
  auto k = gemm_split_pp_kernel<TERMS, F16, EPI, PRO, DEPTH>;
  if (lds > 48 * 1024) {
    static bool attr_set_dev[64] = {};
    int dev = 0;
    (void)hipGetDevice(&dev);
    if (!attr_set_dev[dev & 63]) {
      (void)hipFuncSetAttribute((const void*)k, hipFuncAttributeMaxDynamicSharedMemorySize, lds);
      attr_set_dev[dev & 63] = true;
    }
  }
  hipLaunchKernelGGL(k, dim3(p.per_xcd * 8), dim3(256), (size_t)lds, st, p);
}

template <int TERMS, bool F16>
static void pp_launch_mode(const GemmSplitArgs& p, int pro, bool fused, hipStream_t st) {
  if (pro == 2) pp_launch_one<TERMS, F16, false, 2, 2>(p, st);
  else if (pro == 1) pp_launch_one<TERMS, F16, false, 1, 1>(p, st);
  else if (pro == 3) pp_launch_one<TERMS, F16, false, 3, 1>(p, st);
  else if (fused) pp_launch_one<TERMS, F16, true, 0, 2>(p, st);
  else pp_launch_one<TERMS, F16, false, 0, 2>(p, st);
}

#ifdef SEA_GEMM_KNOCKOUT
template <int KO>
static void ko_launch(const GemmSplitArgs& p, hipStream_t st) {
  constexpr int lds = 2 * 2 * 2 * GS_IMG + 2 * GS_BM * (int)sizeof(float);
  auto k = gemm_split_pp_kernel<2, true, false, 0, 2, KO>;
  (void)hipFuncSetAttribute((const void*)k, hipFuncAttributeMaxDynamicSharedMemorySize, lds);
  hipLaunchKernelGGL(k, dim3(p.per_xcd * 8), dim3(256), (size_t)lds, st, p);
}
extern "C" int sea_gemm_pp_knockout(const float* A, int64_t lda, const void* Wp, float* C, int64_t ldc, int M, int N, int K, int batch,
                                    int64_t strideA, int64_t strideW_bytes, int64_t strideC, const uint32_t* amax_bits, int amax_rows,
                                    int ko, void* stream) {
  GemmSplitArgs p = {};
  p.A = A; p.W = (const char*)Wp; p.C = C; p.lda = lda; p.ldc = ldc; p.strideA = strideA; p.strideW = strideW_bytes; p.strideC = strideC;
  p.M = M; p.N = N; p.K = K; p.Npad = (N + GS_BN - 1) / GS_BN * GS_BN;
  p.mblocks = (M + GS_BM - 1) / GS_BM; p.nblocks = p.Npad / GS_BN; p.total = p.mblocks * p.nblocks * batch; p.per_xcd = (p.total + 7) / 8;
  p.amax_bits = amax_bits; p.amax_rows = amax_rows; p.amax_mul = 1.f;
  p.w_inv = (const float*)((const char*)Wp + (int64_t)(K / GS_BK) * 2 * p.Npad * GS_BK * 2);
  p.ko = ko;
  const hipStream_t st = (hipStream_t)stream;
  switch (ko & ~6) {
    case 0: ko_launch<32>(p, st); break;
    case 1: ko_launch<1>(p, st); break;
    case 8: ko_launch<8>(p, st); break;
    case 9: ko_launch<9>(p, st); break;
    case 16: ko_launch<16>(p, st); break;
    case 24: ko_launch<24>(p, st); break;
    case 25: ko_launch<25>(p, st); break;
    case 64: ko_launch<64>(p, st); break;
    case 72: ko_launch<72>(p, st); break;
    case 128: ko_launch<128>(p, st); break;
    case 129: ko_launch<129>(p, st); break;
    default: return 1;
  }
  return (int)hipGetLastError();
}
#endif

bool gemm_split_pp_launch(const GemmSplitArgs& p, int terms, int pro, bool fused, hipStream_t st) {
  if (p.ldc >= (1ll << 28) || p.ld_add >= (1ll << 28)) return false;
  if (terms == 22) pp_launch_mode<2, true>(p, pro, fused, st);
  else if (terms == 2) pp_launch_mode<2, false>(p, pro, fused, st);
  else if (terms == 1) pp_launch_mode<1, false>(p, pro, fused, st);
  else return false;
  return true;
}

}
```

robust-segmentation_amd/semseg/_native.py:

```python
from __future__ import annotations

import ctypes as C
import os
from typing import Optional

import torch

_PKG = os.path.dirname(os.path.dirname(os.path.abspath(__file__)))
LIB_PATH = os.environ.get("SEA_HIP_LIB", os.path.join(_PKG, "lib", "libsea_hip.so"))

MODE_BY_NAME = {"mask-ce-avg": 0, "mask-ce-bal": 1, "js-avg": 2, "ce": 3, "ce-avg": 3}
DTYPE_CODE = {torch.float32: 0, torch.bfloat16: 1, torch.float16: 2}
LAYOUT_NCHW, LAYOUT_NHWC = 0, 1

_lib = None

_vp, _i, _i64, _f, _sz = C.c_void_p, C.c_int, C.c_int64, C.c_float, C.c_size_t
_SIGS = {
    "sea_abi_version": (C.c_int, []),
    "sea_build_info": (C.c_char_p, []),
    "sea_fastdiv_magic": (_i, [C.c_uint32, C.POINTER(C.c_uint32), C.POINTER(C.c_uint32)]),
    "sea_apgd_linf_step": (_i, [_vp, _vp, _vp, _vp, _vp, _f, _f, _vp, _i, _i64, _vp]),
    "sea_apgd_l2_workspace_bytes": (_i64, [_i]),
    "sea_apgd_l2_step": (_i, [_vp, _vp, _vp, _vp, _vp, _f, _f, _vp, _vp, _i, _i64, _vp]),
    "sea_linf_random_start": (_i, [_vp, _vp, _f, _vp, _i64, _vp]),
    "sea_linf_project": (_i, [_vp, _vp, _f, _vp, _i64, _vp]),
    "sea_pgd_linf_step": (_i, [_vp, _vp, _vp, _f, _f, _vp, _vp, _i, _i64, _vp]),
    "sea_loss_workspace_bytes": (_sz, [_i, _i64]),
    "sea_loss_fwd_bwd": (_i, [_vp, _i, _i, _vp, _i, _vp, _i, _i, _i, _i, _i64, _f, _vp, _vp, _i, _vp, _vp, _sz,
                              _vp, _vp, _vp, _vp]),
    "sea_loss_fwd_bwd_tuned": (_i, [_vp, _i, _i, _vp, _i, _vp, _i, _i, _i, _i, _i64, _f, _vp, _vp, _i, _vp, _vp,
                                    _sz, _vp, _vp, _vp, _vp, _i]),
    "sea_loss_upsampled_workspace_bytes": (_sz, [_i, _i, _i, _i, _i, _i]),
    "sea_loss_fwd_bwd_upsampled": (_i, [_vp, _vp, _i, _vp, _i, _i, _i, _i, _i, _i, _i, _i, _f, _vp, _vp, _i, _vp, _sz, _vp,
                                        _vp, _vp, _vp]),
    "sea_class_counts": (_i, [_vp, _i, _vp, _i, _i, _i, _i64, _i, _i, _vp, _vp, _vp, _vp]),
    "sea_confusion": (_i, [_vp, _i, _vp, _i, _i64, _i, _vp, _vp]),
    "sea_apgd_track": (_i, [_vp, _vp, _vp, _vp, _i, _i64, _i, _i, _i, _i, _i, _vp, _vp, _vp, _vp, _vp, _vp, _vp,
                            _vp, _vp, _vp, _vp]),
    "sea_apgd_linf_step_graph": (_i, [_vp, _vp, _vp, _vp, _vp, _f, _vp, _i, _i64, _vp]),
    "sea_apgd_track_graph": (_i, [_vp, _vp, _vp, _vp, _i, _i64, _vp, _vp, _i, _i, _vp, _vp, _vp, _vp, _vp, _vp, _vp, _vp,
                                  _vp, _vp, _vp]),
    "sea_apgd_linf_step_graph_dev": (_i, [_vp, _vp, _vp, _vp, _vp, _vp, _vp, _i, _i64, _vp]),
    "sea_apgd_track_graph_dev": (_i, [_vp, _vp, _vp, _vp, _i, _i64, _vp, _vp, _vp, _i, _vp, _vp, _vp, _vp, _vp, _vp, _vp, _vp,
                                      _vp, _vp, _vp]),
    "sea_select_copy": (_i, [_vp, _vp, _vp, _vp, _vp, _vp, _vp, _vp, _i, _i, _i64, _i64, _vp]),
    "sea_count_ignored": (_i, [_vp, _i, _i, _i64, _vp, _vp]),
    "sea_worst_miou_greedy": (_i, [_vp, _vp, _i, _i, _i, _vp, _i, _vp, _vp, _vp]),
    "sea_dwconv7x7": (_i, [_vp, _vp, _vp, _vp, _i, _i, _i, _i, _i, _vp]),
    "sea_dwconv7x7_nhwc": (_i, [_vp, _vp, _vp, _vp, _i, _i, _i, _i, _i, _vp]),
    "sea_dwconv7x7_nhwc_add": (_i, [_vp, _vp, _vp, _vp, _vp, _i, _i, _i, _i, _i, _vp]),
    "sea_nchw_to_nhwc": (_i, [_vp, _vp, _vp, _i, _i, _i64, _vp]),
    "sea_nhwc_to_nchw": (_i, [_vp, _vp, _vp, _vp, _i, _i, _i64, _vp]),
    "sea_upsample_bilinear_fwd": (_i, [_vp, _vp, _i64, _i, _i, _i, _i, _vp]),
    "sea_upsample_bilinear_bwd": (_i, [_vp, _vp, _i64, _i, _i, _i, _i, _vp]),
    "sea_layernorm_fwd": (_i, [_vp, _vp, _vp, _vp, _vp, _vp, _i64, _i, _f, _vp]),
    "sea_layernorm_bwd": (_i, [_vp, _vp, _vp, _vp, _vp, _vp, _i64, _i, _vp]),
    "sea_dwconv7x7_nhwc_wgrad_workspace": (_i64, [_i, _i, _i]),
    "sea_dwconv7x7_nhwc_wgrad": (_i, [_vp, _vp, _vp, _vp, _vp, _i, _i, _i, _i, _vp]),
    "sea_adaptive_avg_pool_nhwc_fwd": (_i, [_vp, _vp, _i, _i, _i, _i, _i, _i, _vp]),
    "sea_adaptive_avg_pool_nhwc_bwd": (_i, [_vp, _vp, _i, _i, _i, _i, _i, _i, _vp]),
    "sea_stem_conv1_ln_gelu": (_i, [_vp, _vp, _vp, _vp, _vp, _vp, _vp, _i, _i, _i, _i, _f, _vp]),
    "sea_stem_conv1_bwd": (_i, [_vp, _vp, _vp, _i, _i, _i, _i, _vp]),
    "sea_ln_gelu_cl_fwd": (_i, [_vp, _vp, _vp, _vp, _i, _i, _i, _i64, _f, _vp]),
    "sea_ln_gelu_cl_bwd": (_i, [_vp, _i, _vp, _vp, _vp, _vp, _i, _i, _i64, _f, _vp]),
    "sea_wino_tiles": (_i64, [_i, _i, _i, _i]),
    "sea_wino_input_transform": (_i, [_vp, _i64, _vp, _vp, _vp, _i64, _i, _i, _i, _i, _i, _vp]),
    "sea_wino_filter_transform": (_i, [_vp, _vp, _i, _i, _i, _i, _vp]),
    "sea_wino_output_transform": (_i, [_vp, _vp, _vp, _vp, _i, _vp, _i, _i, _i, _i, _i, _vp]),
    "sea_tap_gather_fwd": (_i, [_vp, _vp, _i, _i, _i, _i, _i, _i, _i, _vp]),
    "sea_tap_gather_bwd": (_i, [_vp, _vp, _i, _i, _i, _i, _i, _i, _vp]),
    "sea_gate_scale": (_i, [_vp, _vp, _vp, _vp, _i64, _i, _vp]),
    "sea_upsample_bilinear_nhwc_fwd": (_i, [_vp, _vp, _vp, _i, _i, _i, _i, _i, _i, _i64, _vp]),
    "sea_upsample_bilinear_nhwc_bwd": (_i, [_vp, _vp, _i, _i, _i, _i, _i, _i, _i64, _vp]),
    "sea_patch2x2": (_i, [_vp, _vp, _i, _i, _i, _i, _i, _vp]),
    "sea_attention_fwd": (_i, [_vp, _vp, _vp, _i64, _i64, _i64, _i, _i, _i, _i, _f, _vp, _vp, _vp]),
    "sea_attention_bwd": (_i, [_vp, _vp, _vp, _i64, _i64, _i64, _i, _i, _i, _i, _f, _vp, _vp, _vp, _vp, _vp, _vp, _vp,
                               _i64, _i64, _i64, _vp]),
    "sea_attention_bwd_terms": (_i, [_vp, _vp, _vp, _i64, _i64, _i64, _i, _i, _i, _i, _f, _vp, _vp, _vp, _vp, _vp, _vp, _vp,
                                     _i64, _i64, _i64, _i, _vp]),
    "sea_attention_fwd_terms": (_i, [_vp, _vp, _vp, _i64, _i64, _i64, _i, _i, _i, _i, _f, _vp, _vp, _i, _vp]),
    "sea_attention_fwd_f16": (_i, [_vp, _vp, _vp, _i64, _i64, _i64, _i, _i, _i, _i, _f, _vp, _vp, _vp, _vp]),
    "sea_attention_bwd_f16": (_i, [_vp, _vp, _vp, _i64, _i64, _i64, _i, _i, _i, _i, _f, _vp, _vp, _vp, _vp, _vp, _vp, _vp, _vp,
                                   _i64, _i64, _i64, _vp]),
    "sea_absmax_bits": (_i, [_vp, _i64, _i, _i, _i, _i64, _i, _vp, _vp]),
    "sea_gemm_split_f16": (_i, [_vp, _i64, _vp, _vp, _i64, _vp, _i, _i, _i, _i, _i, _i64, _i64, _i64, _vp, _i, _vp, _vp]),
    "sea_wino_input_transform_amax": (_i, [_vp, _i64, _vp, _vp, _vp, _i64, _i, _i, _i, _i, _i, _vp, _vp]),
    "sea_gemm_split_fused": (_i, [_vp, _i64, _vp, _vp, _i64, _vp, _i, _i, _i, _i, _i, _i, _i64, _i64, _i64, _vp, _i, _vp, _vp, _vp]),
    "sea_gemm_splitk_reduce": (_i, [_vp, _i, _i, _i, _vp, _vp, _i64, _i, _vp, _i64, _vp, _vp]),
    "sea_gemm_split_packed_bytes": (_i64, [_i, _i, _i]),
    "sea_gemm_split_pack": (_i, [_vp, _i64, _i, _i, _i, _i, _vp, _vp]),
    "sea_gemm_split": (_i, [_vp, _i64, _vp, _vp, _i64, _vp, _i, _i, _i, _i, _i, _i, _i64, _i64, _i64, _vp]),
    "sea_mlp_fused_supported": (_i, [_i, _i]),
    "sea_classifier_supported": (_i, [_i, _i, _i]),
    "sea_classifier_fwd": (_i, [_vp, _vp, _vp, _vp, _i, _i, _i, _i, _vp]),
    "sea_classifier_bwd": (_i, [_vp, _vp, _vp, _i, _i, _i, _i, _vp, _vp, _vp]),
    "sea_probe_gelu_mismatches": (_i, [_vp, _vp]),
    "sea_probe_ln_rows": (_i, [_vp, _vp, _vp, _f, _i, _i, _vp, _vp, _vp, _vp]),
    "sea_mlp_fused_stamps": (_i, [_i, _vp, _i64, _vp, _i64, _vp, _vp, _vp, _vp, _vp, _vp, _vp, _i, _i, _vp, _vp, _vp, _vp, _vp]),
    "sea_mlp_fused_fwd": (_i, [_vp, _i64, _vp, _vp, _vp, _vp, _vp, _i64, _vp, _i64, _i, _i, _i, _vp, _vp, _vp]),
    "sea_mlp_fused_bwd": (_i, [_vp, _i64, _vp, _i64, _vp, _vp, _vp, _vp, _vp, _i64, _i, _i, _i, _vp, _vp, _vp]),
    "sea_ln_mlp_fused_fwd": (_i, [_vp, _i64, _vp, _vp, _f, _vp, _vp, _vp, _vp, _vp, _i64, _vp, _i64, _i, _i, _i, _vp, _vp, _vp]),
    "sea_ln_mlp_fused_bwd": (_i, [_vp, _i64, _vp, _i64, _vp, _vp, _f, _vp, _vp, _vp, _vp, _vp, _i64, _i, _i, _i, _vp, _vp, _vp]),
    "sea_gemm_split_mfma_shape": (_i, [_i]),
    "sea_gemm_split_pipeline": (_i, [_i]),
    "sea_probe_stream_copy": (_i, [_vp, _vp, _sz, _i, _vp]),
    "sea_probe_stream_read": (_i, [_vp, _vp, _sz, _vp]),
    "sea_msf_resize_input": (_i, [_vp, _vp, _vp, _i64, _i, _i, _i, _i, _vp]),
    "sea_msf_accumulate": (_i, [_vp, _vp, _i, _i, _i, _i, _i, _i, _i, _i, _i, _vp]),
    "sea_psp_polyphase_split": (_i, [_vp, _vp, _i, _i, _i, _i, _i, _i, _vp]),
    "sea_psp_polyphase_merge": (_i, [_vp, _vp, _i, _i, _i, _i, _i, _i, _vp]),
    "sea_psp_upsample_ac": (_i, [_vp, _vp, _i64, _i, _i, _i, _i, _vp]),
    "sea_psp_upsample_ac_bwd": (_i, [_vp, _vp, _vp, _i64, _i, _i, _i, _i, _vp]),
    "sea_psp_upsample_ac_nhwc": (_i, [_vp, _vp, _i, _i, _i, _i, _i, _i, _i, _vp]),
    "sea_psp_upsample_ac_nhwc_bwd": (_i, [_vp, _vp, _vp, _i, _i, _i, _i, _i, _i, _i, _vp]),
    "sea_psp_add_relu": (_i, [_vp, _vp, _vp, _i64, _vp]),
    "sea_psp_add_relu_bwd": (_i, [_vp, _vp, _vp, _i64, _vp]),
    "sea_bn_train_workspace_floats": (_i64, [_i64, _i]),
    "sea_bn_train_fwd": (_i, [_vp, _vp, _vp, _vp, _vp, _vp, _vp, _vp, _vp, _vp, _vp, _vp, _i64, _i, _f, _f, _i, _vp]),
    "sea_bn_train_bwd": (_i, [_vp, _vp, _vp, _vp, _vp, _vp, _vp, _vp, _vp, _vp, _vp, _i64, _i, _i, _vp]),
}
EXPORTS = tuple(_SIGS)


class SeaNativeError(RuntimeError):
    pass


def lib():
    global _lib
    if _lib is None:
        if not os.path.exists(LIB_PATH):
            raise SeaNativeError(
                f"libsea_hip.so not found at {LIB_PATH}: build it with "
                "`python robust-segmentation_amd/build_native.py` (there is no CPU fallback)")
        h = C.CDLL(LIB_PATH)
        for name, (res, args) in _SIGS.items():
            fn = getattr(h, name)
            fn.restype, fn.argtypes = res, args
        _lib = h
    return _lib


def _check(rc: int, what: str):
    if rc != 0:
        raise SeaNativeError(f"{what} failed with hipError {rc}")


def _dev(*ts):
    cur = None
    for t in ts:
        if t is None:
            continue
        if not t.is_cuda:
            raise SeaNativeError("libsea_hip works on HIP device tensors only (no CPU fallback); got a CPU tensor")
        if cur is None:
            cur = torch.cuda.current_device()
        if t.device.index != cur:
            raise SeaNativeError(f"tensor on {t.device} but the current device is cuda:{cur}: call "
                                 "torch.cuda.set_device (or use `with torch.cuda.device(...)`) before the launch")


def _stream() -> int:
    return torch._C._cuda_getCurrentRawStream(torch.cuda.current_device())


_K2_FORCE = int(os.environ.get("SEA_K2_FORCE", "0"), 0)


def _p(t: Optional[torch.Tensor]):
    return None if t is None else t.data_ptr()

# ... 792 lines not shown
    qkv = _f32c(qkv)
    B, T, three, H, D = qkv.shape
    if three != 3 or D != 64:
        raise SeaNativeError("attention_qkv expects a (B,T,3,H,64) tensor")
    out = torch.empty(B, T, H * D, dtype=torch.float32, device=qkv.device)
    lse = torch.empty(B, H, T, dtype=torch.float32, device=qkv.device)
    p = qkv.data_ptr()
    terms = attn_terms_fwd() if terms is None else int(terms)
    if terms == 22:
        ws = torch.empty(4 * B * H, dtype=torch.int32, device=qkv.device)
        _check(lib().sea_attention_fwd_f16(p, p + 4 * H * D, p + 8 * H * D, T * 3 * H * D, D, 3 * H * D, B, H, T, D, float(scale),
                                           _p(ws), _p(out), _p(lse), _stream()), "sea_attention_fwd_f16")
        return out, lse
    _check(lib().sea_attention_fwd_terms(p, p + 4 * H * D, p + 8 * H * D, T * 3 * H * D, D, 3 * H * D, B, H, T, D, float(scale),
                                         _p(out), _p(lse), terms, _stream()), "sea_attention_fwd_terms")
    return out, lse


ATTN_TERMS_BWD_DEFAULT = 22


def attn_terms_bwd() -> int:
    t = int(os.environ.get("SEA_ATTN_TERMS_BWD", ATTN_TERMS_BWD_DEFAULT))
    return t if t in (0, 2, 3, 22) else ATTN_TERMS_BWD_DEFAULT


ATTN_TERMS_FWD_DEFAULT = 22


def attn_terms_fwd() -> int:
    t = int(os.environ.get("SEA_ATTN_TERMS", ATTN_TERMS_FWD_DEFAULT))
    return t if t in (0, 2, 3, 22) else ATTN_TERMS_FWD_DEFAULT


def attention_qkv_backward(qkv, out, lse, grad_out, scale: float, terms=None):
    _dev(qkv, out, lse, grad_out)
    B, T, _, H, D = qkv.shape
    grad_out = _f32c(grad_out.contiguous())
    dqkv = torch.empty_like(qkv)
    delta = torch.empty_like(lse)
    p, g = qkv.data_ptr(), dqkv.data_ptr()
    sb, sh, st = T * 3 * H * D, D, 3 * H * D
    terms = attn_terms_bwd() if terms is None else int(terms)
    head = (p, p + 4 * H * D, p + 8 * H * D, sb, sh, st, B, H, T, D, float(scale), _p(_f32c(out)), _p(grad_out),
            _p(_f32c(lse)), _p(delta))
    tail = (g, g + 4 * H * D, g + 8 * H * D, sb, sh, st)
    if terms == 22:
        ws = torch.empty(4 * B * H, dtype=torch.int32, device=qkv.device)
        _check(lib().sea_attention_bwd_f16(*head, _p(ws), *tail, _stream()), "sea_attention_bwd_f16")
    else:
        _check(lib().sea_attention_bwd_terms(*head, *tail, terms, _stream()), "sea_attention_bwd_terms")
    return dqkv


def worst_miou_greedy(ints: torch.Tensor, unions: torch.Tensor, mt_state, n_rounds: int = 1000):
    import numpy as np
    A, N, Cc = ints.shape
    ti = np.ascontiguousarray(ints.detach().cpu().numpy(), dtype=np.float32)
    tu = np.ascontiguousarray(unions.detach().cpu().numpy(), dtype=np.float32)
    mt = np.array(mt_state, dtype=np.uint32)
    assert mt.shape == (625,)
    sel = np.zeros(N, dtype=np.int32)
    miou = C.c_double(0.0)
    rounds = C.c_int32(0)
    rc = lib().sea_worst_miou_greedy(ti.ctypes.data, tu.ctypes.data, A, N, Cc, mt.ctypes.data, n_rounds,
                                     C.addressof(miou), sel.ctypes.data, C.addressof(rounds))
    _check(rc, "sea_worst_miou_greedy")
    return miou.value, sel.tolist(), rounds.value, tuple(int(v) for v in mt)


CACHE_EPOCH = [0]


class PackedWeight:

    def __init__(self, data, N, K, terms, batch, src=None):
        self.data, self.N, self.K, self.terms, self.batch = data, N, K, terms, batch
        self.stride = data.numel() // batch
        self.src = src
        self.slices = {}

    def _slices_of(self, S):
        W, trans = self.src
        Ws = W.view(S, self.K // S, self.N) if trans else W.view(self.N, S, self.K // S).permute(1, 0, 2)
        return gemm_split_pack(Ws, trans=trans, terms=self.terms)

    def k_slices(self, S):
        if S not in self.slices:
            self.slices[S] = self._slices_of(S)
            CACHE_EPOCH[0] += 1
        return self.slices[S]

    def refresh_from(self, new) -> bool:
        if (self.data.shape != new.data.shape or (self.N, self.K, self.terms, self.batch) != (new.N, new.K, new.terms, new.batch)
                or (self.src is None) != (new.src is None)):
            return False
        self.data.copy_(new.data)
        self.src = new.src
        for S, sl in self.slices.items():
            sl.data.copy_(self._slices_of(S).data)
        return True


def gemm_split_pack(W, trans: bool = False, terms: int = 3) -> PackedWeight:
    _dev(W)
    if W.dtype != torch.float32 or W.dim() not in (2, 3) or W.stride(-1) != 1:
        raise SeaNativeError("gemm_split_pack: float32 (N,K) / (G,N,K) weights with a contiguous last dim expected")
    Wb = W if W.dim() == 3 else W.unsqueeze(0)
    G = Wb.shape[0]
    N, K = (Wb.shape[2], Wb.shape[1]) if trans else (Wb.shape[1], Wb.shape[2])
    L = lib()
    nbytes = L.sea_gemm_split_packed_bytes(N, K, terms)
    if nbytes < 0:
        raise SeaNativeError(f"gemm_split_pack: unsupported shape N={N} K={K} terms={terms} (K % 32 == 0, terms 1, 2, 3 or 22)")
    out = torch.empty(G, nbytes, dtype=torch.uint8, device=W.device)
    for g in range(G):
        _check(L.sea_gemm_split_pack(_p(Wb[g]), Wb.stride(1), int(trans), N, K, terms, _p(out[g]), _stream()),
               "sea_gemm_split_pack")
    return PackedWeight(out, N, K, terms, G, src=(W.detach(), trans) if (W.dim() == 2 and W.is_contiguous()) else None)


USE_MLP_FUSED = os.environ.get("SEA_MLP_FUSED", "1") != "0"
USE_CLASSIFIER = os.environ.get("SEA_CLASSIFIER", "1") != "0"


def classifier_ok(P: int, K: int, cls: int) -> bool:
    return bool(USE_CLASSIFIER and lib().sea_classifier_supported(int(P), int(K), int(cls)))


def classifier_forward(y_rows, w2d, bias, B: int, P: int):
    _dev(y_rows, w2d, bias)
    cls, K = w2d.shape
    if (y_rows.dtype != torch.float32 or y_rows.shape != (B * P, K) or not y_rows.is_contiguous() or y_rows.data_ptr() % 16
            or w2d.dtype != torch.float32 or not w2d.is_contiguous() or w2d.data_ptr() % 16
            or (bias is not None and (bias.dtype != torch.float32 or bias.numel() != cls or not bias.is_contiguous()))):
        raise SeaNativeError("classifier_forward: y (B P, K) / W (cls, K) must be contiguous, 16-byte aligned float32")
    out = torch.empty((B, cls, P), dtype=torch.float32, device=y_rows.device)
    _check(lib().sea_classifier_fwd(_p(y_rows), _p(w2d), _p(bias), _p(out), B, P, K, cls, _stream()), "sea_classifier_fwd")
    return out


def classifier_backward(g, w2d, gate=None, gate_scale=None):
    _dev(g, w2d, gate, gate_scale)
    cls, K = w2d.shape
    if (gate is None) != (gate_scale is None):
        raise SeaNativeError("classifier_backward: gate and gate_scale come together")
    if gate is not None and (gate.dtype != torch.float32 or gate.dim() != 2 or gate.shape[1] != K or not gate.is_contiguous()
                             or gate_scale.dtype != torch.float32 or gate_scale.numel() != K or not gate_scale.is_contiguous()
                             or g.dim() != 3 or gate.shape[0] != g.shape[0] * g.shape[2]):
        raise SeaNativeError("classifier_backward: gate must be contiguous float32 (B P, K) rows, gate_scale (K)")
    if (g.dtype != torch.float32 or g.dim() != 3 or g.shape[1] != cls or not g.is_contiguous()
            or w2d.dtype != torch.float32 or not w2d.is_contiguous() or w2d.data_ptr() % 16):
        raise SeaNativeError("classifier_backward: g (B, cls, P) / W (cls, K) must be contiguous float32")
    B, _, P = g.shape
    gy = torch.empty((B * P, K), dtype=torch.float32, device=g.device)
    _check(lib().sea_classifier_bwd(_p(g), _p(w2d), _p(gy), B, P, K, cls, _p(gate), _p(gate_scale), _stream()), "sea_classifier_bwd")
    return gy


def mlp_fused_ok(C: int, H: int) -> bool:
    return bool(USE_MLP_FUSED and lib().sea_mlp_fused_supported(int(C), int(H)))


def _mlp_rows(t, C, what):
    if t.dtype != torch.float32 or t.dim() != 2 or t.shape[1] != C or t.stride(1) != 1 or t.stride(0) % 4 or t.data_ptr() % 16:
        raise SeaNativeError(f"mlp_fused: {what} must be float32 (M, {C}) rows, 16-byte aligned, row stride % 4 == 0")


def _ln_args(ln, Cc):
    if ln is None:
        return None
    w, b, eps = ln
    if (w.dtype != torch.float32 or b.dtype != torch.float32 or w.numel() != Cc or b.numel() != Cc or not w.is_contiguous()
            or not b.is_contiguous() or w.data_ptr() % 16 or b.data_ptr() % 16):
        raise SeaNativeError("mlp_fused: LayerNorm weight / bias must be contiguous, 16-byte aligned float32 of C entries")
    return w, b, float(eps)


def mlp_fused_forward(x2, W1p: PackedWeight, b1, W2p: PackedWeight, b2, res, amax_x, amax_h, out=None, ln=None):
    _dev(x2, b1, b2, res, out, amax_x, amax_h, *(ln[:2] if ln is not None else ()))
    M, Cc = x2.shape
    H = W1p.N
    if (W1p.terms, W2p.terms, W1p.K, W2p.N, W2p.K, W1p.batch, W2p.batch) != (22, 22, Cc, Cc, H, 1, 1):
        raise SeaNativeError("mlp_fused_forward: fp16 x 2 packs of w1 (H x C) and w2 (C x H) expected")
    _mlp_rows(x2, Cc, "x")
    if res is not None:
        _mlp_rows(res, Cc, "res")
    if out is None:
        out = torch.empty(M, Cc, dtype=torch.float32, device=x2.device)
    _mlp_rows(out, Cc, "out")
    la = _ln_args(ln, Cc)
    if la is not None:
        _check(lib().sea_ln_mlp_fused_fwd(_p(x2), x2.stride(0), _p(la[0]), _p(la[1]), la[2], _p(W1p.data), _p(b1), _p(W2p.data),
                                          _p(b2), _p(res), res.stride(0) if res is not None else 0, _p(out), out.stride(0), M, Cc,
                                          H, _p(amax_x), _p(amax_h), _stream()), "sea_ln_mlp_fused_fwd")
        return out
    _check(lib().sea_mlp_fused_fwd(_p(x2), x2.stride(0), _p(W1p.data), _p(b1), _p(W2p.data), _p(b2), _p(res),
                                   res.stride(0) if res is not None else 0, _p(out), out.stride(0), M, Cc, H, _p(amax_x),
                                   _p(amax_h), _stream()), "sea_mlp_fused_fwd")
    return out


def mlp_fused_backward(g2, x2, W1p: PackedWeight, b1, W2tp: PackedWeight, W1tp: PackedWeight, amax_x, amax_mul, out=None,
                       ln=None):
    _dev(g2, x2, b1, out, amax_x, amax_mul)
    M, Cc = x2.shape
    H = W1p.N
    if ((W1p.terms, W2tp.terms, W1tp.terms) != (22, 22, 22) or (W1p.K, W2tp.N, W2tp.K, W1tp.N, W1tp.K) != (Cc, H, Cc, Cc, H)
            or amax_mul.dtype != torch.float32 or amax_mul.numel() != 1):
        raise SeaNativeError("mlp_fused_backward: fp16 x 2 packs of w1, w2^T, w1^T and one float32 amax_mul expected")
    _mlp_rows(x2, Cc, "x")
    _mlp_rows(g2, Cc, "g")
    if out is None:
        out = torch.empty(M, Cc, dtype=torch.float32, device=x2.device)
    _mlp_rows(out, Cc, "out")
    la = _ln_args(ln, Cc)
    if la is not None:
        _dev(*la[:2])
        _check(lib().sea_ln_mlp_fused_bwd(_p(g2), g2.stride(0), _p(x2), x2.stride(0), _p(la[0]), _p(la[1]), la[2], _p(W1p.data),
                                          _p(b1), _p(W2tp.data), _p(W1tp.data), _p(out), out.stride(0), M, Cc, H, _p(amax_x),
                                          _p(amax_mul), _stream()), "sea_ln_mlp_fused_bwd")
        return out
    _check(lib().sea_mlp_fused_bwd(_p(g2), g2.stride(0), _p(x2), x2.stride(0), _p(W1p.data), _p(b1), _p(W2tp.data),
                                   _p(W1tp.data), _p(out), out.stride(0), M, Cc, H, _p(amax_x), _p(amax_mul), _stream()),
           "sea_mlp_fused_bwd")
    return out


class AmaxPool:
    _pools = {}
    SIZE = 1024

    def __init__(self, device):
        self.buf = torch.zeros(self.SIZE, dtype=torch.int32, device=device)
        self.next = 0

    @classmethod
    def get(cls, device):
        device = torch.device(device)
        key = (device.type, device.index if device.index is not None else torch.cuda.current_device())
        if key not in cls._pools:
            cls._pools[key] = AmaxPool(device)
        return cls._pools[key]

    def reset(self):
        self.buf.zero_()
        self.next = 0

    def word(self):
        if self.next >= self.SIZE:
            self.buf = torch.zeros(self.SIZE, dtype=torch.int32, device=self.buf.device)
            self.next = 0
        w = self.buf[self.next:self.next + 1]
        self.next += 1
        return w


AMAX_FROM_PRODUCERS = os.environ.get("SEA_AMAX_FUSE", "1") != "0"


def amax_word(device):
    return AmaxPool.get(device).word()


KSPLIT = os.environ.get("SEA_GEMM_KSPLIT", "1") != "0"
KSPLIT_BELOW, KSPLIT_TARGET, KSPLIT_MIN_KB = (int(v) for v in os.environ.get("SEA_GEMM_KSPLIT_PARAMS", "400,768,8").split(","))
_ksplit_ws = {}


def _ksplit(M, N, K):
    blocks = -(-M // 128) * -(-N // 128)
    nkb = K // 32
    if not KSPLIT or blocks >= KSPLIT_BELOW or N % 4:
        return 1
    S = min(-(-KSPLIT_TARGET // blocks), nkb // KSPLIT_MIN_KB)
    while S > 1 and nkb % S:
        S -= 1
    return max(S, 1)


def _ksplit_workspace(device, numel):
    key = device.index if device.index is not None else torch.cuda.current_device()
    ws = _ksplit_ws.get(key)
    if ws is None or ws.numel() < numel:
        ws = _ksplit_ws[key] = torch.empty(numel, dtype=torch.float32, device=device)
    return ws[:numel]


def ksplit_workspace_pin(device):
    return _ksplit_ws.get(device.index if device.index is not None else torch.cuda.current_device())


class _GemmEpilogue(C.Structure):
    _fields_ = [("addend", C.c_void_p), ("ld_addend", C.c_int64), ("stride_addend", C.c_int64),
                ("gelu_out", C.c_void_p), ("gelu_grad_of", C.c_void_p), ("a_gelu_grad_of", C.c_void_p), ("a_gate", C.c_int), ("a_gelu", C.c_int),
                ("a_amax_mul", C.c_float), ("a_amax_mul_dev", C.c_void_p)]


def _amax_words(A3, M, K, G, sA, groups, per_row=False):
    if per_row and G != 1:
        raise SeaNativeError("gemm_split: row_amax (one scale word per row) is defined for a single matrix, not a batch of them")
    if per_row:
        words = torch.empty(M, dtype=torch.int32, device=A3.device)
        _check(lib().sea_absmax_bits(_p(A3), A3.stride(1), M, K, 1, 0, 1, _p(words), _stream()), "sea_absmax_bits")
        return words, 1
    rpw = M // groups if (groups > 1 and M % groups == 0) else 0
    words = torch.empty(groups if rpw else 1, dtype=torch.int32, device=A3.device)
    _check(lib().sea_absmax_bits(_p(A3), A3.stride(1), M, K, G, sA, rpw, _p(words), _stream()), "sea_absmax_bits")
    return words, rpw


def gemm_split(A, Wp: PackedWeight, bias=None, relu: bool = False, out=None, amax=None, out_amax=None, addend=None,
               gelu_out=None, gelu_grad_of=None, amax_rows: int = 0, groups: int = 1, a_gelu_grad_of=None,
               a_gelu: bool = False, a_relu_gate=None, row_amax: bool = False, amax_mul: float = 1.0):
    gate = a_relu_gate is not None
    if gate:
        if a_gelu_grad_of is not None:
            raise SeaNativeError("gemm_split: a_relu_gate and a_gelu_grad_of are exclusive")
        a_gelu_grad_of = a_relu_gate
    _dev(A, bias, out, addend, gelu_out, gelu_grad_of, a_gelu_grad_of)
    batched = Wp.batch > 1 or A.dim() == 3
    A3 = A if A.dim() == 3 else A.unsqueeze(0)
    if (A.dtype != torch.float32 or A3.dim() != 3 or A3.shape[0] != Wp.batch or A3.shape[2] != Wp.K
            or A3.stride(2) != 1):
        raise SeaNativeError("gemm_split: A must be float32 (M,K) / (G,M,K) with K matching the packed weights")
    G, M, K = A3.shape
    if out is None:
        out = torch.empty((G, M, Wp.N) if batched else (M, Wp.N), dtype=torch.float32, device=A.device)
    O3 = out if out.dim() == 3 else out.unsqueeze(0)
    if O3.shape != (G, M, Wp.N) or O3.stride(2) != 1 or out.dtype != torch.float32:
        raise SeaNativeError("gemm_split: output must be float32 (.., M, N) with a contiguous last dim")
    if bias is not None and (bias.dtype != torch.float32 or bias.numel() != Wp.N or not bias.is_contiguous()):
        raise SeaNativeError("gemm_split: bias must be contiguous float32 of N entries")
    sA, sC = (A3.stride(0) if G > 1 else 0), (O3.stride(0) if G > 1 else 0)
    if amax is not None and (amax.dtype != torch.int32 or not amax.is_contiguous()
                             or amax.numel() < (-(-M // amax_rows) if amax_rows > 0 else 1)):
        raise SeaNativeError("gemm_split: amax must hold one int32 word per amax_rows rows")
    mul_dev = amax_mul if (torch.is_tensor(amax_mul) and Wp.terms == 22) else None
    if mul_dev is not None and (mul_dev.dtype != torch.float32 or mul_dev.numel() != 1 or mul_dev.device != A.device):
        raise SeaNativeError("gemm_split: a tensor amax_mul must be one float32 on A's device")
    amax_mul = float(amax_mul) if (Wp.terms == 22 and mul_dev is None) else 1.0
    fused = (addend is not None or gelu_out is not None or gelu_grad_of is not None or a_gelu_grad_of is not None
             or a_gelu or amax_mul != 1.0 or mul_dev is not None)
    if a_gelu_grad_of is not None and (a_gelu_grad_of.shape != A.shape or a_gelu_grad_of.stride() != A.stride()
                                       or a_gelu_grad_of.dtype != torch.float32 or Wp.terms not in (1, 2, 22)):
        raise SeaNativeError("gemm_split: a_gelu_grad_of must be float32 with A's shape and strides (terms 1, 2 or 22)")
    only_pro = gelu_out is None and gelu_grad_of is None
    add_ok = addend is None or (addend.dim() == 2 and addend.shape == O3.shape[1:] and addend.stride(1) == 1
                                and addend.stride(0) % 4 == 0 and addend.data_ptr() % 16 == 0 and addend.dtype == torch.float32)
    if G == 1 and (not fused or (only_pro and add_ok)) and Wp.src is not None and O3.stride(1) % 4 == 0 and O3.data_ptr() % 16 == 0:
        S = _ksplit(M, Wp.N, K)
        if S > 1:
            if Wp.terms == 22 and amax is None:
                amax, amax_rows = _amax_words(A3, M, K, 1, 0, groups, row_amax)
            part = _ksplit_workspace(A.device, S * M * Wp.N).view(S, M, Wp.N)
            shape, strides = (S, M, K // S), (K // S, A3.stride(1), 1)
            gemm_split(A3[0].as_strided(shape, strides), Wp.k_slices(S), out=part, amax=amax, amax_rows=amax_rows,
                       a_gelu_grad_of=None if (a_gelu_grad_of is None or gate) else a_gelu_grad_of.as_strided(shape, strides),
                       a_gelu=a_gelu, amax_mul=mul_dev if mul_dev is not None else amax_mul,
                       **({"a_relu_gate": a_gelu_grad_of.as_strided(shape, strides)} if gate else {}))
            _check(lib().sea_gemm_splitk_reduce(_p(part), S, M, Wp.N, _p(bias), _p(addend),
                                                addend.stride(0) if addend is not None else 0, int(relu), _p(O3), O3.stride(1),
                                                _p(out_amax) if Wp.terms == 22 else None, _stream()), "sea_gemm_splitk_reduce")
            return out
    if addend is not None and (a_gelu or a_gelu_grad_of is not None):
        out = gemm_split(A, Wp, bias=bias, relu=False, out=out, amax=amax, out_amax=None, amax_rows=amax_rows, groups=groups,
                         a_gelu_grad_of=None if gate else a_gelu_grad_of, a_gelu=a_gelu,
                         a_relu_gate=a_gelu_grad_of if gate else None, row_amax=row_amax,
                         amax_mul=mul_dev if mul_dev is not None else amax_mul)
        out += addend
        if relu:
            torch.relu_(out)
        if out_amax is not None and Wp.terms == 22:
            O2 = out if out.dim() == 3 else out.unsqueeze(0)
            _check(lib().sea_absmax_bits(_p(O2), O2.stride(1), M, Wp.N, G, sC, 0, _p(out_amax), _stream()), "sea_absmax_bits")
        return out
    if fused:
        epi = _GemmEpilogue()
        if addend is not None:
            D3 = addend if addend.dim() == 3 else addend.unsqueeze(0)
            if D3.shape != O3.shape or D3.stride(2) != 1 or addend.dtype != torch.float32:
                raise SeaNativeError("gemm_split: addend must be float32 of the output's shape with a contiguous last dim")
            epi.addend, epi.ld_addend, epi.stride_addend = D3.data_ptr(), D3.stride(1), (D3.stride(0) if G > 1 else 0)
        for name, t in (("gelu_out", gelu_out), ("gelu_grad_of", gelu_grad_of)):
            if t is not None:
                T3 = t if t.dim() == 3 else t.unsqueeze(0)
                if T3.shape != O3.shape or T3.stride() != O3.stride() or t.dtype != torch.float32:
                    raise SeaNativeError(f"gemm_split: {name} must be float32 with the output's shape and strides")
                setattr(epi, name, T3.data_ptr())
        if a_gelu_grad_of is not None:
            epi.a_gelu_grad_of = a_gelu_grad_of.data_ptr()
            epi.a_gate = int(gate)
        epi.a_gelu = int(bool(a_gelu))
        epi.a_amax_mul = amax_mul if amax_mul != 1.0 else 0.0
        epi.a_amax_mul_dev = mul_dev.data_ptr() if mul_dev is not None else None
        if Wp.terms == 22 and amax is None:
            amax, amax_rows = _amax_words(A3, M, K, G, sA, groups, row_amax)
        _check(lib().sea_gemm_split_fused(_p(A3), A3.stride(1), _p(Wp.data), _p(O3), O3.stride(1), _p(bias), int(relu), M, Wp.N,
                                          K, Wp.terms, G, sA, Wp.stride, sC, _p(amax) if Wp.terms == 22 else None, amax_rows,
                                          _p(out_amax) if Wp.terms == 22 else None, C.addressof(epi), _stream()),
               "sea_gemm_split_fused")
        return out
    if Wp.terms == 22:
        if amax is None:
            amax, amax_rows = _amax_words(A3, M, K, G, sA, groups, row_amax)
        _check(lib().sea_gemm_split_f16(_p(A3), A3.stride(1), _p(Wp.data), _p(O3), O3.stride(1), _p(bias), int(relu), M, Wp.N,
                                        K, G, sA, Wp.stride, sC, _p(amax), amax_rows, _p(out_amax), _stream()),
               "sea_gemm_split_f16")
        return out
    _check(lib().sea_gemm_split(_p(A3), A3.stride(1), _p(Wp.data), _p(O3), O3.stride(1), _p(bias), int(relu), M, Wp.N, K,
                                Wp.terms, G, sA, Wp.stride, sC, _stream()), "sea_gemm_split")
    return out
```

robust-segmentation_amd/semseg/attacker.py:

```python
from __future__ import annotations

from functools import partial

import os
import weakref

import torch

from . import _native as N

__all__ = [
    "apgd_train", "apgd_largereps", "apgd_restarts", "criterion_dict", "masked_cross_entropy",
    "masked_cross_entropy_balanced", "js_loss", "js_div_fn", "pixel_to_img_loss", "compute_iou_acc",
    "check_oscillation", "Logger",
]


class Logger:

    def __init__(self, log_path=None):
        self.log_path = log_path

    def log(self, str_to_log):
        print(str_to_log)
# ... 408 lines not shown
        N.count_ignored(self.yc, out=own.n_ignored)
        own.reset(self.eps, n_iter, self.cps)
        own.busy = True

    def _loss(self, logits, want_grad):
        o = self.own
        ev = None
        if self.k2_events is not None:
            ev = (torch.cuda.Event(enable_timing=True), torch.cuda.Event(enable_timing=True))
            ev[0].record()
        if self.fused:
            r = N.loss_fwd_bwd_upsampled(logits.detach().contiguous(), self.yc, self.w, self.mode, self.tmode,
                                         self.gscale, want_grad=want_grad, pred=o.pred, workspace=o.k2u_workspace(logits),
                                         out=o.stats, dlow=o.dlogits if want_grad else None)
        else:
            r = N.loss_fwd_bwd(logits.detach(), self.yc, self.w, self.mode, self.tmode, self.gscale,
                               want_grad=want_grad, pred=o.pred, workspace=o.ws, out=o.stats,
                               dlogits=o.dlogits if want_grad else None, defer=self.defer)
        if ev is not None:
            ev[1].record()
            self.k2_events.append(ev)
        if want_grad:
            o.keep_k2_grad(r["dlogits"])
        self.last = r
        return r

    def _select(self):
        o = self.own
        N.select_copy(o.st.flags, self.x_adv, o.grad, o.x_best, o.grad_best, o.x_best_adv, o.pred, o.pred_best)

    def start(self):
        o = self.own
        x_in, logits = _forward_logits(self.model, self.x_adv, True, self.fused)
        r = self._loss(logits, True)
        g = _input_grad(logits, x_in, r["dlogits"])
        del logits
        N.apgd_track(r, o.n_ignored, self.HW, 0, max(self.n_iter, 1), 0, False, True, o.st)
        o.grad.copy_(g)
        o.grad_best.copy_(g)
        o.pred_best.copy_(o.pred)
        for t in (o.x_best, o.x_best_adv, self.x_old):
            t.copy_(self.x_adv)

    def step(self, i: int):
        if self.use_graph:
            if self._first_graph_step <= i < self.n_iter - 1:
                return self._step_graph(i)
            if i == 1:
                cur = torch.cuda.current_stream()
                self._gs.wait_stream(cur)
                with torch.cuda.stream(self._gs):
                    self._step_eager(i)
                cur.wait_stream(self._gs)
                return
        self._step_eager(i)

    def _step_eager(self, i: int):
        o = self.own
        a = 0.75 if i > 0 else 1.0
        if self.norm == "L2":
            if self._l2_ws is None:
                self._l2_ws = torch.empty(N.lib().sea_apgd_l2_workspace_bytes(self.B) // 8, dtype=torch.float64, device=o.x.device)
            N.apgd_l2_step(o.x, self.x_adv, self.x_old, o.grad, o.st.step, self.eps, a, out=self.x_next, workspace=self._l2_ws)
        else:
            N.apgd_linf_step(o.x, self.x_adv, self.x_old, o.grad, o.st.step, self.eps, a, out=self.x_next)
        self.x_old, self.x_adv, self.x_next = self.x_adv, self.x_next, self.x_old
        want = i < self.n_iter - 1
        x_in, logits = _forward_logits(self.model, self.x_adv, want, self.fused)
        r = self._loss(logits, want)
        if want:
            o.grad.copy_(_input_grad(logits, x_in, r["dlogits"]))
        del logits
        N.apgd_track(r, o.n_ignored, self.HW, i, self.n_iter, self.cps.get(i, 0), self.early_stop, False, o.st)
        self._select()

    def _graph_failed(self, exc):
        import sys
        self.use_graph = False
        self.own.drop_graphs()
        torch.cuda.set_stream(self._caller_stream)
        print(f"[sea] HIP-graph capture of the attack step failed ({type(exc).__name__}: {str(exc).splitlines()[0][:160]}); "
              "continuing with the eager loop", file=sys.stderr)
        torch.cuda.synchronize()

    def _capture(self, i: int):
        o = self.own
        self._caller_stream = torch.cuda.current_stream()
        o.it_dev.fill_(i)
        ga, gb = torch.cuda.CUDAGraph(), torch.cuda.CUDAGraph()
        try:
            with torch.cuda.graph(ga, stream=self._gs):
                N.apgd_linf_step_graph(o.x, self.x_adv, self.x_old, o.grad, o.st.step, o.eps_dev, o.it_dev)
                g_xin, g_logits = _forward_logits(self.model, self.x_adv, True, self.fused)
        except Exception as exc:
            self._graph_failed(exc)
            return self._step_eager(i)
        ga.replay()
        r = self._loss(g_logits, True)
        try:
            with torch.cuda.graph(gb, pool=ga.pool(), stream=self._gs):
                o.grad.copy_(_input_grad(g_logits, g_xin, r["dlogits"]))
                N.apgd_track_graph(r, o.n_ignored, self.HW, o.it_dev, o.cp_dev, o.niter_dev, self.early_stop, o.st)
                self._select()
        except Exception as exc:
            self._graph_failed(exc)
            del g_xin, g_logits
            x_in, logits = _forward_logits(self.model, self.x_adv, True, self.fused)
            r = self._loss(logits, True)
            o.grad.copy_(_input_grad(logits, x_in, r["dlogits"]))
            del logits
            N.apgd_track(r, o.n_ignored, self.HW, i, self.n_iter, self.cps.get(i, 0), self.early_stop, False, o.st)
            self._select()
            return
        gb.replay()
        o.keep_graphs((ga, gb), self._graph_sig(), g_xin, g_logits)

    def _graph_sig(self):
        return (bool(self.early_stop), bool(self.defer), _arith_signature(self.model))

    def _step_graph(self, i: int):
        o = self.own
        if o.graphs is not None and i == self._first_graph_step:
            if o.sig != self._graph_sig():
                o.drop_graphs()
            else:
                o.it_dev.fill_(i)
        if o.graphs is None:
            self._capture(i)
            return
        o.graphs[0].replay()
        self._loss(o.g_logits, True)
        o.graphs[1].replay()

    def release_graphs(self):
        if self._private:
            self.own.drop_graphs()
        self.own.busy = False

    def result(self):
        o = self.own
        return o.x_best.clone(), o.st.acc.clone(), o.st.loss_best.clone(), o.x_best_adv.clone()


def apgd_train(model, x, y, norm, eps, n_iter=10, use_rs=False, loss="ce", verbose=False, is_train=False,
               early_stop=False, track_loss=None, logger=None, y_target=None, ignore_index=-1, x_init=None,
               num_classes=21, weights=None, gpuu=None, noise=None, poll_every: int = 8, return_pred: bool = False):
    assert not model.training
    assert ignore_index == -1, "Only `ignore_index = 1` is supported."
    if norm == "L1":
        raise NotImplementedError("the L1 branch of apgd_train (reference semseg/attacker.py:437-454, 553-566: sparse steps, "
                                  "L1_projection, adaptive sparsity) is not built: no entry point of the reference reaches it "
                                  "(SURVEY fact 2; tools/infer.py and tools/train_rob_seg.py pass norm='Linf')")
    if norm not in ("Linf", "L2"):
        raise ValueError(f"norm {norm!r}: 'Linf' or 'L2'")
    if norm == "L2" and use_rs and x_init is None:
        raise ValueError("apgd_train(norm='L2', use_rs=True) needs x_init: the reference draws a random start for L-inf only")
    if loss not in N.MODE_BY_NAME:
        raise KeyError(loss)
    if not x.is_cuda:
        raise N.SeaNativeError("apgd_train needs HIP device tensors (no CPU fallback)")
    device = x.device
    x = x.detach().contiguous().float()

    if not use_rs or norm != "Linf":
        x_adv = x.clone()
    else:
# ... 112 lines not shown
```

robust-segmentation_amd/semseg/models/convnext_upernet.py:

```python
from __future__ import annotations

import os

import torch
import torch.nn.functional as F
from torch import nn

CONVNEXT_SETTINGS = {
    "T": ([3, 3, 9, 3], [96, 192, 384, 768], 384, 0.4),
    "T_CVST": ([3, 3, 9, 3], [96, 192, 384, 768], 384, 0.4),
    "T_CVST_ROB": ([3, 3, 9, 3], [96, 192, 384, 768], 384, 0.4),
    "S_CVST": ([3, 3, 27, 3], [96, 192, 384, 768], 384, 0.3),
    "S_CVST_ROB": ([3, 3, 27, 3], [96, 192, 384, 768], 384, 0.3),
    "B": ([3, 3, 27, 3], [128, 256, 512, 1024], 512, 0.4),
}


def _fp32_fwd(fn):
    def forward(ctx, *args):
        if torch.is_autocast_enabled():
            args = [a.float() if (torch.is_tensor(a) and a.is_floating_point() and a.dtype != torch.float32) else a
                    for a in args]
            with torch.autocast("cuda", enabled=False):
                return fn(ctx, *args)
# ... 233 lines not shown
    if cache.get(name + "_key") != key:
        with torch.no_grad():
            cache[name] = _stable(cache.get(name), N.gemm_split_pack(w.detach(), trans=trans, terms=terms))
        cache[name + "_key"] = key
    return cache[name]


def _frozen_mm(x2d, w, cache, name, trans=False, bias=None, relu=False, terms=None, amax=None, out_amax=None, groups=1,
               row_amax=False):
    K = w.shape[0] if trans else w.shape[1]
    terms = _terms() if terms is None else terms
    if _split_ok(x2d, K, terms):
        from .. import _native as N
        if terms != 22:
            amax = out_amax = None
        return N.gemm_split(x2d, _packed(w, cache, name, trans, terms), bias=bias, relu=relu, amax=amax, out_amax=out_amax,
                            groups=groups, row_amax=row_amax)
    wt = w if trans else w.t()
    y = torch.addmm(bias, x2d, wt) if bias is not None else x2d @ wt
    return torch.relu_(y) if relu else y


def _ln_bound_word(norm, cache):
    key = _tkey(norm.weight, norm.bias)
    if cache.get("ln_bound_key") != key:
        with torch.no_grad():
            bnd = norm.weight.numel() ** 0.5 * norm.weight.abs().max() + norm.bias.abs().max()
            cache.update(ln_bound_key=key, ln_bound=_stable(cache.get("ln_bound"), bnd.float().reshape(1).contiguous().view(torch.int32)))
    return cache["ln_bound"]


def _linear_bound_word(in_word, w, b, cache):
    key = (_tkey(w, b), in_word._version)
    if cache.get("lin_bound_key") != key or cache.get("lin_bound_in") is not in_word:
        with torch.no_grad():
            bnd = in_word.view(torch.float32) * w.abs().sum(1)
            if b is not None:
                bnd = bnd + b.abs()
            cache.update(lin_bound_key=key, lin_bound_in=in_word,
                         lin_bound=_stable(cache.get("lin_bound"), bnd.max().float().reshape(1).contiguous().view(torch.int32)))
    return cache["lin_bound"]


def _l1_bound(w, cache, dim, factor=1.0):
    key = (_tkey(w), dim, factor)
    if cache.get("l1_key") != key:
        with torch.no_grad():
            cache.update(l1_key=key, l1=_stable(cache.get("l1"), (w.detach().abs().sum(dim).max() * (factor * (1.0 + 1e-6))).float().reshape(1)))
    return cache["l1"]


class _FrozenLinear(torch.autograd.Function):

    @staticmethod
    @_fp32_fwd
    def forward(ctx, x, w, b, cache, amax=None, out_amax=None):
        ctx.w, ctx.cache, ctx.shape, ctx.terms = w, cache, x.shape, _terms()
        x2 = x.reshape(-1, x.shape[-1])
        return _frozen_mm(x2, w, cache, "lin_fwd", bias=b, amax=amax, out_amax=out_amax,
                          groups=x.shape[0] if x.dim() > 2 else 1).view(*x.shape[:-1], w.shape[0])

    @staticmethod
    @_fp32_bwd
    def backward(ctx, gy):
        g2 = gy.reshape(-1, gy.shape[-1])
        if not g2.is_contiguous():
            g2 = g2.contiguous()
        return (_frozen_mm(g2, ctx.w, ctx.cache, "lin_bwd", trans=True, terms=_bwd_terms(ctx.terms), row_amax=True,
                           groups=ctx.shape[0] if len(ctx.shape) > 2 else 1).view(ctx.shape), None, None, None, None, None)


def _linear_frozen(mod_cache, x, w, b, amax=None, out_amax=None):
    if (_terms() in (1, 2, 3, 22) and x.is_cuda and x.dtype == torch.float32 and not w.requires_grad
            and (b is None or not b.requires_grad) and w.shape[1] % 32 == 0 and not torch.is_autocast_enabled()
            and x.is_contiguous() and x.numel() // x.shape[-1] >= GEMM_MIN_ROWS):
        return _FrozenLinear.apply(x, w, b, mod_cache, amax, out_amax)
    return F.linear(x, w, b)


FUSE_MLP = int(os.environ.get("SEA_FUSE_MLP", "24"))
RELU_GATE_PROLOGUE = os.environ.get("SEA_RELU_GATE_PROLOGUE", "1") != "0"
REDUCE_ADD = os.environ.get("SEA_REDUCE_ADD", "1") != "0"
FUSE_PROLOGUE_MAX_NBLOCKS = int(os.environ.get("SEA_FUSE_PRO_NB", "3"))


def _mlp_fusable(x, w1, b1, w2, b2):
    return (FUSE_MLP >= 0 and _terms() in (1, 2, 3, 22) and x.is_cuda and x.dtype == torch.float32 and x.is_contiguous()
            and not torch.is_autocast_enabled() and x.numel() // x.shape[-1] >= GEMM_MIN_ROWS
            and w1.shape[1] % 32 == 0 and w2.shape[1] % 32 == 0 and w2.shape[0] == x.shape[-1]
            and not any(t is not None and t.requires_grad for t in (w1, b1, w2, b2)))


class _FrozenMlp(torch.autograd.Function):

    @staticmethod
    @_fp32_fwd
    def forward(ctx, x, w1, b1, w2, b2, res, caches, a1, a2, ln=None):
        from .. import _native as N
        terms = _terms()
        x2 = x.reshape(-1, x.shape[-1])
        ctx.ln = None
        if terms != 22:
            a1 = a2 = None
        fuse, nb = int(FUSE_MLP), (x.shape[0] if x.dim() > 2 else 1)
        r2 = None if res is None else res.reshape(-1, res.shape[-1])
        ctx.w, ctx.b1, ctx.caches, ctx.shape, ctx.terms, ctx.has_res = (w1, w2), b1, caches, x.shape, terms, res is not None
        ctx.fuse, ctx.a1 = fuse, a1
        rows_ok = lambda t: t.stride(1) == 1 and t.stride(0) % 4 == 0 and t.data_ptr() % 16 == 0
        if (terms == 22 and fuse & 16 and a1 is not None and a2 is not None and a1.numel() == 1 and a2.numel() == 1
                and b1 is not None and N.mlp_fused_ok(w2.shape[0], w1.shape[0]) and rows_ok(x2)
                and (r2 is None or rows_ok(r2))):
            y = N.mlp_fused_forward(x2, _packed(w1, caches[0], "lin_fwd", False, terms), b1,
                                    _packed(w2, caches[1], "lin_fwd", False, terms), b2, r2, a1, a2, ln=ln)
            ctx.kernel_fused, ctx.ln = True, ln
            ctx.save_for_backward(x2)
            return y.view(x.shape)
        if ln is not None:
            raise RuntimeError("_FrozenMlp: a LayerNorm was handed in but the fused kernel does not apply (see _mlp_takes_layernorm)")
        ctx.kernel_fused = False
        t = torch.empty(x2.shape[0], w1.shape[0], dtype=torch.float32, device=x.device)
        pro = bool(fuse & 16) and -(-w2.shape[0] // 128) <= FUSE_PROLOGUE_MAX_NBLOCKS and not fuse & 1
        if pro:
            N.gemm_split(x2, _packed(w1, caches[0], "lin_fwd", False, terms), bias=b1, out=t, amax=a1, groups=nb)
            h = t
        elif fuse & 1:
            h = torch.empty_like(t)
            N.gemm_split(x2, _packed(w1, caches[0], "lin_fwd", False, terms), bias=b1, out=t, gelu_out=h, amax=a1, groups=nb)
        else:
            N.gemm_split(x2, _packed(w1, caches[0], "lin_fwd", False, terms), bias=b1, out=t, amax=a1, groups=nb)
            h = F.gelu(t)
        split2 = REDUCE_ADD and N._ksplit(x2.shape[0], w2.shape[0], w2.shape[1]) > 1
        add_in = r2 is not None and r2.is_contiguous() and (split2 or (bool(fuse & 4) and not pro))
        y = N.gemm_split(t if pro else h, _packed(w2, caches[1], "lin_fwd", False, terms), bias=b2, amax=a2, groups=nb,
                         a_gelu=pro, addend=r2 if add_in else None)
        if r2 is not None and not add_in:
            y += r2
        ctx.save_for_backward(t)
        return y.view(x.shape)

    @staticmethod
    @_fp32_bwd
    def backward(ctx, g):
        from .. import _native as N
        (t,) = ctx.saved_tensors
        terms = _bwd_terms(ctx.terms)
        g2 = g.reshape(-1, g.shape[-1])
        if not g2.is_contiguous():
            g2 = g2.contiguous()
        nb = ctx.shape[0] if len(ctx.shape) > 2 else 1
        if ctx.kernel_fused:
            x2 = t
            p1f = _packed(ctx.w[0], ctx.caches[0], "lin_fwd", False, ctx.terms)
            if terms == 22 and g2.data_ptr() % 16 == 0:
                gx = N.mlp_fused_backward(g2, x2, p1f, ctx.b1, _packed(ctx.w[1], ctx.caches[1], "lin_bwd", True, terms),
                                          _packed(ctx.w[0], ctx.caches[0], "lin_bwd", True, terms), ctx.a1,
                                          _l1_bound(ctx.w[1], ctx.caches[1], dim=0, factor=1.13), ln=ctx.ln)
                return gx.view(ctx.shape), None, None, None, None, (g if ctx.has_res else None), None, None, None, None
            if ctx.ln is not None:
                xin = x2
                x2, ln_mean, ln_rstd = N.layernorm(xin, ctx.ln[0], ctx.ln[1], ctx.ln[2])
            t = N.gemm_split(x2, p1f, bias=ctx.b1, amax=ctx.a1, groups=nb)
        p2, p1 = (_packed(ctx.w[1], ctx.caches[1], "lin_bwd", True, terms), _packed(ctx.w[0], ctx.caches[0], "lin_bwd", True, terms))
        rows = {}
        if terms == 22:
            words, _ = N._amax_words(g2.unsqueeze(0), g2.shape[0], g2.shape[1], 1, 0, nb, per_row=True)
            rows = dict(amax=words, amax_rows=1)
            mul = dict(amax_mul=_l1_bound(ctx.w[1], ctx.caches[1], dim=0, factor=1.13), **rows)
        else:
            mul = {}
        if ctx.fuse & 2:
            gx = N.gemm_split(N.gemm_split(g2, p2, gelu_grad_of=t, groups=nb, **rows), p1, groups=nb, **mul)
        elif ctx.fuse & 8 and terms in (1, 2, 22) and -(-ctx.w[0].shape[1] // 128) <= FUSE_PROLOGUE_MAX_NBLOCKS:
            gx = N.gemm_split(N.gemm_split(g2, p2, groups=nb, **rows), p1, a_gelu_grad_of=t, groups=nb, **mul)
        else:
            gx = N.gemm_split(torch.ops.aten.gelu_backward(N.gemm_split(g2, p2, groups=nb, **rows), t), p1, groups=nb, **mul)
        if ctx.kernel_fused and ctx.ln is not None:
            gx = N.layernorm_backward(gx.contiguous(), xin, ctx.ln[0], ln_mean, ln_rstd)
        return gx.view(ctx.shape), None, None, None, None, (g if ctx.has_res else None), None, None, None, None


def _mlp_takes_layernorm(y, norm, w1, b1, w2, a1, a2):
    from .. import _native as N
    return (FUSE_LN_INTO_MLP and _terms() == 22 and int(FUSE_MLP) & 16 and a1 is not None and a2 is not None and a1.numel() == 1
            and a2.numel() == 1 and b1 is not None and N.mlp_fused_ok(w2.shape[0], w1.shape[0]) and y.is_contiguous()
            and y.data_ptr() % 16 == 0 and norm.weight is not None and norm.bias is not None
            and not (norm.weight.requires_grad or norm.bias.requires_grad) and norm.weight.is_contiguous()
            and norm.bias.is_contiguous() and norm.weight.data_ptr() % 16 == 0 and norm.bias.data_ptr() % 16 == 0
            and USE_HIP_LAYERNORM and _bwd_terms(22) == 22)


FUSE_LN_INTO_MLP = os.environ.get("SEA_MLP_FUSE_LN", "1") != "0"


def _taps_major(conv: nn.Conv2d):
    w = conv.weight
    key = _tkey(w)
    cached = getattr(conv, "_sea_wt", None)
    if cached is None or cached[0] != key:
        cached = (key, _stable(None if cached is None else cached[1], w.detach().reshape(w.shape[0], 49).t().contiguous()))
        conv._sea_wt = cached
    return cached[1]


def depthwise7x7(conv: nn.Conv2d, x):
    if x.is_cuda and x.dtype == torch.float32 and conv.weight.dtype == torch.float32 and USE_HIP_DWCONV:
        return _DwConv7x7.apply(x, conv.weight, conv.bias)
    return conv(x)


USE_HIP_DWCONV = True
LN_CONTIGUOUS = os.environ.get("SEA_LN_CONTIGUOUS", "0") != "0"


class _ToNHWC(torch.autograd.Function):

    @staticmethod
    @_fp32_fwd
    def forward(ctx, x):
        from .. import _native as N
        return N.nchw_to_nhwc(x)

    @staticmethod
    @_fp32_bwd
    def backward(ctx, g):
        from .. import _native as N
        return N.nhwc_to_nchw(g.contiguous())


class _ScaleResidual(torch.autograd.Function):

    @staticmethod
    @_fp32_fwd
    def forward(ctx, x, y, gamma):
        from .. import _native as N
        ctx.save_for_backward(y if (gamma is not None and gamma.requires_grad) else None, gamma)
        return N.nhwc_to_nchw(y, gamma, x)

    @staticmethod
    @_fp32_bwd
    def backward(ctx, g):
        from .. import _native as N
        y, gamma = ctx.saved_tensors
        g = g.contiguous()
        gx = g if ctx.needs_input_grad[0] else None
        gy = N.nchw_to_nhwc(g, gamma) if ctx.needs_input_grad[1] else None
        gg = None
        if gamma is not None and ctx.needs_input_grad[2]:
            gg = (N.nchw_to_nhwc(g) * y).sum((0, 1, 2))
        return gx, gy, gg


USE_HIP_TRANSPOSE = True
STAGE_ENTRY_CONTIGUOUS = False


def _fast_layout_ok(x):
# ... 825 lines not shown
```

robust-segmentation_amd/semseg/val.py:

```python
from __future__ import annotations

import math
import os
import sys
import weakref

import torch

from . import _native as N
from . import attacker as _A
from .attacker import _FrozenParameters
from .metrics import Metrics

__all__ = ["Pgd_Attack", "Pgd_Attack_1", "evaluate", "evaluate_msf", "msf_scaled_size", "losses", "js_loss",
           "masked_cross_entropy"]


def js_loss(p, q, reduction="mean"):
    return _A.js_loss(p, q, reduction=reduction)


def masked_cross_entropy(pred, target):
    return _A.masked_cross_entropy(pred, target, reduction="mean")

# ... 61 lines not shown
    for m in ([model] if model is not None else list(_PGD_SLOTS.keys())):
        _PGD_SLOTS.pop(m, None)


class Pgd_Attack_1:

    def __init__(self, epsilon=4.0 / 255.0, alpha=1e-2, num_iter=2, los="pgd"):
        self.epsilon, self.alpha, self.num_iter, self.los_name = epsilon, alpha, num_iter, los
        self.loss_fn = losses[los]
        self.mode, self.per_image = self.loss_fn.mode, self.loss_fn.per_image

    def adv_attack(self, model, X, y, delta0=None):
        model.eval()
        X = X.detach().contiguous().float()
        B, HW = X.shape[0], X.shape[-2] * X.shape[-1]
        y = _labels(y) if self.mode is not None else y
        delta = torch.zeros_like(X).uniform_(-self.epsilon, self.epsilon) if delta0 is None else delta0.clone()
        scale = 1.0 / (HW if self.per_image else B * HW)
        ws = N.loss_workspace(B, HW, X.device)
        out = tuple(torch.empty(B, dtype=d, device=X.device) for d in (torch.float32, torch.float32, torch.int32))
        if (PGD_GRAPH and self.mode is not None and self.num_iter >= PGD_GRAPH_MIN_ITER and X.is_cuda
                and isinstance(model, torch.nn.Module)):
            res = self._adv_attack_graph(model, X, y, delta, scale)
            if res is not None:
                return res
        x_in = X + delta
        logits, dl = None, None
        for _ in range(self.num_iter):
            g, r, logits = _fwd_grad(model, x_in, y, self.loss_fn, scale, ws, out, dl)
            dl = r["dlogits"]
            N.pgd_linf_step(X, delta, g, float(self.alpha), float(self.epsilon), delta_out=delta, x_in_out=x_in,
                            clamp_input=False)
        x_adv = (X + delta).clamp_(0.0, 1.0)
        return x_adv.detach(), logits, None

    def _adv_attack_graph(self, model, X, y, delta, scale):
        try:
            slots = _PGD_SLOTS.setdefault(model, {})
        except TypeError:
            return None
        ac = (torch.is_autocast_enabled(), torch.get_autocast_dtype("cuda") if torch.is_autocast_enabled() else None)
        key = (tuple(X.shape), tuple(y.shape), y.dtype, X.device.index, self.mode, self.per_image, float(self.alpha),
               float(self.epsilon), ac)
        sl = slots.get(key)
        if sl is None:
            sl = slots[key] = _PgdSlot(X, y)
        if sl.failed:
            return None
        sl.X.copy_(X)
        sl.y.copy_(y)
        sl.delta.copy_(delta)
        torch.add(sl.X, sl.delta, out=sl.x_in)
        alpha, eps = float(self.alpha), float(self.epsilon)

        def iteration():
            g, r, logits = _fwd_grad(model, sl.x_in, sl.y, self.loss_fn, scale, sl.ws, sl.out, sl.dl)
            sl.dl = r["dlogits"]
            N.pgd_linf_step(sl.X, sl.delta, g, alpha, eps, delta_out=sl.delta, x_in_out=sl.x_in, clamp_input=False)
            return logits

        logits = iteration()
        wkey = _param_key(model)
        if sl.graph is not None and (sl.epoch != N.CACHE_EPOCH[0] or sl.wkey != wkey):
            sl.graph = sl.logits = sl.pin = None
        it = 1
        cur = torch.cuda.current_stream()
        gs = _A._capture_stream(X.device)
        if sl.graph is None:
            if not sl.warm:
                gs.wait_stream(cur)
                with torch.cuda.stream(gs):
                    logits = iteration()
                cur.wait_stream(gs)
                sl.warm = True
                it += 1
            if it < self.num_iter:
                graph = torch.cuda.CUDAGraph()
                try:
                    with torch.cuda.graph(graph, stream=gs):
                        sl.logits = iteration()
                except Exception as exc:
                    torch.cuda.set_stream(cur)
                    torch.cuda.synchronize()
                    sl.failed = True
                    print(f"[sea] HIP-graph capture of the inner PGD failed ({type(exc).__name__}: "
                          f"{str(exc).splitlines()[0][:160]}); continuing with the eager loop", file=sys.stderr)
                    for _ in range(it, self.num_iter):
                        logits = iteration()
                    return (sl.X + sl.delta).clamp_(0.0, 1.0).detach(), logits, None
                sl.graph, sl.epoch, sl.wkey = graph, N.CACHE_EPOCH[0], wkey
                sl.pin = N.ksplit_workspace_pin(X.device)
        for _ in range(it, self.num_iter):
            sl.graph.replay()
            logits = sl.logits
        x_adv = (sl.X + sl.delta).clamp_(0.0, 1.0)
        return x_adv.detach(), (logits.clone() if logits is not None else None), None


class Pgd_Attack:

    def __init__(self, eps=4.0 / 255.0, alpha=1e-2, num_iter=2, los="pgd", epsilon=None):
        self.epsilon = eps if epsilon is None else epsilon
        self.alpha, self.num_iter, self.los_name = alpha, num_iter, los
        self.loss_fn = losses[los]
        self.mode, self.per_image = self.loss_fn.mode, self.loss_fn.per_image
        if not self.per_image:
            raise ValueError("Pgd_Attack needs a per-image loss ('mask-ce-avg' or 'js-avg'); use Pgd_Attack_1 for 'pgd'")

    def adv_attack(self, model, X, y, wt=None):
        model.eval()
        X = X.detach().contiguous().float()
        B, HW = X.shape[0], X.shape[-2] * X.shape[-1]
        y = _labels(y) if self.mode is not None else y.long()
        delta = torch.zeros_like(X)
        best_delta = torch.zeros_like(X)
        best = torch.zeros(B, device=X.device)
        ws = N.loss_workspace(B, HW, X.device)
        out = tuple(torch.empty(B, dtype=d, device=X.device) for d in (torch.float32, torch.float32, torch.int32))
        x_in = X.clamp(0.0, 1.0)
        dl = None
        for _ in range(self.num_iter):
            g, r, _ = _fwd_grad(model, x_in, y, self.loss_fn, 1.0 / HW, ws, out, dl)
            dl = r["dlogits"]
            loss = r["loss_img"] if "loss_img" in r else r["loss_sum"] / HW
            ind = loss >= best
            best = torch.where(ind, loss, best)
            N.pgd_linf_step(X, delta, g, float(self.alpha), float(self.epsilon), delta_out=delta, x_in_out=x_in,
                            clamp_input=True)
            best_delta = torch.where(ind.view(-1, 1, 1, 1), delta, best_delta)
        return (X + best_delta).clamp_(0.0, 1.0).detach(), None, None


@torch.no_grad()
def evaluate(model, dataloader, device, cls, n_batches=-1):
    model.eval()
    metrics = Metrics(cls, -1, device)
    for i, batch in enumerate(dataloader):
        images, labels = batch[0].to(device), batch[1].to(device)
        metrics.update(model(images), labels)
        if i + 1 == n_batches:
            break
    ious, miou = metrics.compute_iou()
    cla_acc, macc, aacc = metrics.compute_pixel_acc()
    f1, mf1 = metrics.compute_f1()
    return cla_acc, macc, aacc, f1, mf1, ious, miou


def msf_scaled_size(scale, H, W):
    return int(math.ceil(int(scale * H) / 32)) * 32, int(math.ceil(int(scale * W) / 32)) * 32


_MSF_SCORE = weakref.WeakKeyDictionary()


def _msf_logits(model, x):
    if hasattr(model, "forward_lowres"):
        r = model.forward_lowres(x)
        if isinstance(r, (tuple, list)):
            r = r[0]
        if torch.is_tensor(r):
            return r.float().contiguous()
    return model(x).float().contiguous()


def _score_buffer(model, shape, device):
    try:
# ... 52 lines not shown
```

Measured before the change: 563.4.

## Fuse split-K reduction into GEMM via last-arriving-block fixup with counters

Adds an in-kernel split-K fix-up: each K-slice block writes its partial tile, bumps a per-tile atomic counter, and the last arriving block sums all slices and applies bias, addend, relu, GELU or GELU-gradient and amax. This removes the separate split-K reduce launch and lets batched (grouped) GEMMs and the MLP GELU paths use split-K too, optionally ordering slices so siblings land on different XCDs. The cost is extra threadfences and atomics, counter state that must be reset after failed graph capture, and partial-buffer traffic still being read back.

Result: no change. 562.7 (-0.1%).

```diff
diff --git a/include/sea_hip.h b/include/sea_hip.h
--- a/include/sea_hip.h
+++ b/include/sea_hip.h
@@ -180,6 +180,23 @@
 int sea_gemm_split_pack(const float* W, int64_t ldw, int trans, int N, int K, int terms, void* out, void* stream);
 int sea_gemm_splitk_reduce(const float* partial, int splits, int M, int N, const float* bias, const float* addend,
                            int64_t ld_addend, int relu, float* C, int64_t ldc, uint32_t* out_amax, void* stream);
+struct SeaGemmEpilogue;
+typedef struct SeaSplitKFixup {
+  int splits, slice_order, relu, n_counters;
+  int64_t strideA_group;
+  float* C;
+  int64_t ldc, strideC;
+  const float* bias;
+  const float* addend;
+  int64_t ld_addend, stride_addend;
+  uint32_t* out_amax;
+  float* gelu_out;
+  const float* gelu_grad_of;
+  int* counters;
+} SeaSplitKFixup;
+int sea_gemm_split_ksliced(const float* A, int64_t lda, const void* Wp_slices, float* partial, int M, int N, int K_slice,
+                           int terms, int groups, int64_t strideA_slice, int64_t strideW_bytes, const uint32_t* amax_bits,
+                           int amax_rows, const struct SeaGemmEpilogue* epi, const SeaSplitKFixup* fx, void* stream);
 typedef struct SeaGemmEpilogue {
   const float* addend;
   int64_t ld_addend, stride_addend;
diff --git a/robust-segmentation_amd/csrc/gemm_split.h b/robust-segmentation_amd/csrc/gemm_split.h
--- a/robust-segmentation_amd/csrc/gemm_split.h
+++ b/robust-segmentation_amd/csrc/gemm_split.h
@@ -87,12 +87,50 @@
   int a_gelu;
   int a_gate;
   int ko;
+  int fx_S;
+  int fx_order;
+  int fx_relu;
+  int64_t fx_strideA_grp;
+  float* fx_C;
+  int64_t fx_ldc, fx_strideC;
+  const float* fx_bias;
+  const float* fx_addend;
+  int64_t fx_ld_add, fx_stride_add;
+  uint32_t* fx_out_amax;
+  float* fx_gelu_out;
+  const float* fx_gelu_grad_of;
+  int* fx_counters;
 };
+
+__device__ __forceinline__ int64_t gemm_split_a_off(const GemmSplitArgs& p, int g) {
+  if (p.fx_S > 1) return (int64_t)(g / p.fx_S) * p.fx_strideA_grp + (int64_t)(g % p.fx_S) * p.strideA;
+  return (int64_t)g * p.strideA;
+}
+
+__device__ __forceinline__ void gemm_split_tile_of(const GemmSplitArgs& p, int logical, int& g, int& mb, int& nb) {
+  int s = 0;
+  const bool by_slice = p.fx_S > 1 && p.fx_order;
+  if (by_slice) {
+    s = logical % p.fx_S;
+    logical /= p.fx_S;
+  }
+  nb = logical % p.nblocks;
+  const int t2 = logical / p.nblocks;
+  mb = t2 % p.mblocks;
+  g = t2 / p.mblocks;
+  if (by_slice) g = g * p.fx_S + s;
+}
 
 __device__ __forceinline__ float gelu_f(float x) { return 0.5f * x * (1.f + erff(x * 0.70710678118654752440f)); }
 __device__ __forceinline__ float gelu_grad_f(float x) {
   const float cdf = 0.5f * (1.f + erff(x * 0.70710678118654752440f));
   const float pdf = __expf(-0.5f * x * x) * 0.39894228040143267794f;
+  return cdf + x * pdf;
+}
+
+__device__ __forceinline__ float gelu_grad_exact_f(float x) {
+  const float cdf = 0.5f * (1.f + erff(x * 0.70710678118654752440f));
+  const float pdf = expf(-0.5f * x * x) * 0.39894228040143267794f;
   return cdf + x * pdf;
 }
 
@@ -195,6 +233,75 @@
   }
 }
 
+template <int BM, int BN, int NT>
+__device__ __forceinline__ void gemm_split_fixup(const GemmSplitArgs& p, int g, int mb, int nb) {
+  const int S = p.fx_S;
+  const int grp = g / S;
+  __shared__ int fx_last;
+  __syncthreads();
+  if (threadIdx.x == 0) {
+    __threadfence();
+    int* const word = p.fx_counters + ((int64_t)grp * p.mblocks + mb) * p.nblocks + nb;
+    const int last = atomicAdd(word, 1) == S - 1;
+    if (last) atomicExch(word, 0);
+    fx_last = last;
+  }
+  __syncthreads();
+  if (!fx_last) return;
+  __threadfence();
+  const int M = p.M, N = p.N;
+  const int m0 = mb * BM, n0 = nb * BN;
+  const int64_t ldp = p.ldc, sp = p.strideC, ldc = p.fx_ldc, ld_add = p.fx_ld_add;
+  const float* const part = p.C + (int64_t)grp * S * sp;
+  float* const Cg = p.fx_C + (int64_t)grp * p.fx_strideC;
+  const float* const bias = p.fx_bias;
+  const float* const addg = p.fx_addend ? p.fx_addend + (int64_t)grp * p.fx_stride_add : nullptr;
+  float* const gelu_out = p.fx_gelu_out ? p.fx_gelu_out + (int64_t)grp * p.fx_strideC : nullptr;
+  const float* const gelu_src = p.fx_gelu_grad_of ? p.fx_gelu_grad_of + (int64_t)grp * p.fx_strideC : nullptr;
+  const int relu = p.fx_relu;
+  constexpr int F4 = BN / 4;
+  uint32_t omax = 0;
+  for (int i = threadIdx.x; i < BM * F4; i += NT) {
+    const int rl = i / F4, c4 = i - rl * F4;
+    const int row = m0 + rl, col = n0 + 4 * c4;
+    if (row >= M || col >= N) continue;
+    const float* const pp = part + (int64_t)row * ldp + col;
+    f32x4 v = *(const f32x4*)pp;
+    for (int s = 1; s < S; ++s) v += *(const f32x4*)(pp + (int64_t)s * sp);
+    if (bias) v += *(const f32x4*)(bias + col);
+    if (addg) v += *(const f32x4*)(addg + (int64_t)row * ld_add + col);
+    if (relu) {
+#pragma unroll
+      for (int e = 0; e < 4; ++e) v[e] = v[e] > 0.f ? v[e] : 0.f;
+    }
+    if (gelu_src) {
+      const f32x4 t = *(const f32x4*)(gelu_src + (int64_t)row * ldc + col);
+#pragma unroll
+      for (int e = 0; e < 4; ++e) v[e] *= gelu_grad_exact_f(t[e]);
+    }
+    *(f32x4*)(Cg + (int64_t)row * ldc + col) = v;
+    if (gelu_out) {
+      f32x4 o;
+#pragma unroll
+      for (int e = 0; e < 4; ++e) o[e] = gelu_f(v[e]);
+      *(f32x4*)(gelu_out + (int64_t)row * ldc + col) = o;
+    }
+#pragma unroll
+    for (int e = 0; e < 4; ++e) {
+      const uint32_t vb = __float_as_uint(v[e]) & 0x7fffffffu;
+      omax = vb > omax ? vb : omax;
+    }
+  }
+  if (p.fx_out_amax != nullptr) {
+#pragma unroll
+    for (int o = 32; o > 0; o >>= 1) {
+      const uint32_t other = (uint32_t)__shfl_xor((int)omax, o, 64);
+      omax = other > omax ? other : omax;
+    }
+    if ((threadIdx.x & 63) == 0 && omax > *(volatile uint32_t*)p.fx_out_amax) atomicMax(p.fx_out_amax, omax);
+  }
+}
+
 bool gemm_split_pp_launch(const GemmSplitArgs& p, int terms, int pro, bool fused, hipStream_t st);
 bool gemm_split_big_launch(GemmSplitArgs p, int terms, int batch, int shape, int pro, hipStream_t st);
 
diff --git a/robust-segmentation_amd/csrc/gemm_split.hip b/robust-segmentation_amd/csrc/gemm_split.hip
--- a/robust-segmentation_amd/csrc/gemm_split.hip
+++ b/robust-segmentation_amd/csrc/gemm_split.hip
@@ -12,10 +12,8 @@
   const int64_t lda = p.lda, ldc = p.ldc;
   const int logical = (int)(blockIdx.x & 7) * p.per_xcd + (int)(blockIdx.x >> 3);
   if ((int)(blockIdx.x >> 3) >= p.per_xcd || logical >= p.total) return;
-  const int nb = logical % p.nblocks;
-  const int t2 = logical / p.nblocks;
-  const int mb = t2 % p.mblocks;
-  const int g = t2 / p.mblocks;
+  int g, mb, nb;
+  gemm_split_tile_of(p, logical, g, mb, nb);
   const int m0 = mb * GS_BM, n0 = nb * GS_BN;
   const float* const w_inv = F16 ? (const float*)((const char*)p.w_inv + (int64_t)g * p.strideW) : nullptr;
 
@@ -24,7 +22,7 @@
   const int r = lane & 31, h = lane >> 5;
 
   const int q = tid & 7, arow = tid >> 3;
-  const char* const Abase = (const char*)(p.A + (int64_t)g * p.strideA);
+  const char* const Abase = (const char*)(p.A + gemm_split_a_off(p, g));
   float* const Cbase = p.C;
   const float* const bias = p.bias;
   const int64_t strideC = p.strideC;
@@ -66,7 +64,7 @@
 
   f32x4 pa[4];
   f32x4 pt[(PRO == 1 || PRO == 3) ? 4 : 1];
-  const char* const Tbase = (PRO == 1 || PRO == 3) ? (const char*)(p.a_gelu_grad_of + (int64_t)g * p.strideA) : nullptr;
+  const char* const Tbase = (PRO == 1 || PRO == 3) ? (const char*)(p.a_gelu_grad_of + gemm_split_a_off(p, g)) : nullptr;
   u32x4 pw[2 * TERMS];
   auto fetch = [&](int kb) {
     const char* a = Abase + (int64_t)kb * (GS_BK * 4);
@@ -180,6 +178,7 @@
       __syncthreads();
     }
     gemm_split_store_tile<F16, EPI>(p, acc, g, m0, n0, smem, row_inv, bv_c, wi_c);
+    if (p.fx_S > 1) gemm_split_fixup<GS_BM, GS_BN, 256>(p, g, mb, nb);
   } else {
     const int r16 = lane & 15, c16 = lane >> 4;
     f32x4v acc[4][4];
@@ -268,6 +267,7 @@
       }
       if (lane == 0 && omax16 > *(volatile uint32_t*)p.out_amax) atomicMax(p.out_amax, omax16);
     }
+    if (p.fx_S > 1) gemm_split_fixup<GS_BM, GS_BN, 256>(p, g, mb, nb);
   }
 }
 
@@ -558,7 +558,7 @@
 static int gemm_split_impl(const float* A, int64_t lda, const void* Wp, float* C, int64_t ldc, const float* bias, int relu, int M,
                            int N, int K, int terms, int batch, int64_t strideA, int64_t strideW_bytes, int64_t strideC,
                            const uint32_t* amax_bits, int amax_rows, uint32_t* out_amax, void* stream,
-                           const SeaGemmEpilogue* epi = nullptr);
+                           const SeaGemmEpilogue* epi = nullptr, const SeaSplitKFixup* fx = nullptr);
 
 extern "C" int sea_gemm_split(const float* A, int64_t lda, const void* Wp, float* C, int64_t ldc, const float* bias,
                               int relu, int M, int N, int K, int terms, int batch, int64_t strideA, int64_t strideW_bytes,
@@ -591,6 +591,27 @@
   }
   return gemm_split_impl(A, lda, Wp, C, ldc, bias, relu, M, N, K, terms, batch, strideA, strideW_bytes, strideC,
                          terms == 22 ? amax_bits : nullptr, amax_rows, out_amax, stream, epi);
+}
+
+extern "C" int sea_gemm_split_ksliced(const float* A, int64_t lda, const void* Wp_slices, float* partial, int M, int N, int K_slice,
+                                      int terms, int groups, int64_t strideA_slice, int64_t strideW_bytes,
+                                      const uint32_t* amax_bits, int amax_rows, const SeaGemmEpilogue* epi,
+                                      const SeaSplitKFixup* fx, void* stream) {
+  SEA_CHECK_ARG(terms == 1 || terms == 2 || terms == 3 || (terms == 22 && amax_bits != nullptr && amax_rows >= 0));
+  SEA_CHECK_ARG(fx && partial && fx->C && fx->counters && fx->splits > 1 && groups > 0 && M > 0 && N > 0);
+  SEA_CHECK_ARG((int64_t)groups * fx->splits < (1 << 20) && (N % 4) == 0 && fx->ldc >= N && (fx->ldc % 4) == 0 && (fx->strideC % 4) == 0);
+  SEA_CHECK_ARG(((((uintptr_t)partial) | ((uintptr_t)fx->C) | ((uintptr_t)fx->bias) | ((uintptr_t)fx->addend) |
+                  ((uintptr_t)fx->gelu_out) | ((uintptr_t)fx->gelu_grad_of)) & 15) == 0);
+  SEA_CHECK_ARG(!fx->addend || (fx->ld_addend >= N && (fx->ld_addend % 4) == 0 && (fx->stride_addend % 4) == 0));
+  SEA_CHECK_ARG(!(fx->gelu_out && fx->gelu_grad_of) && !(fx->relu && (fx->gelu_out || fx->gelu_grad_of)));
+  SEA_CHECK_ARG(terms == 22 || fx->out_amax == nullptr);
+  SEA_CHECK_ARG((fx->strideA_group % 4) == 0);
+  SEA_CHECK_ARG((int64_t)groups * ((M + GS_BM - 1) / GS_BM) * ((N + GS_BN - 1) / GS_BN) <= fx->n_counters);
+  if (epi) {
+    SEA_CHECK_ARG(!epi->addend && !epi->gelu_out && !epi->gelu_grad_of && !(epi->a_gelu_grad_of && epi->a_gelu));
+  }
+  return gemm_split_impl(A, lda, Wp_slices, partial, N, nullptr, 0, M, N, K_slice, terms, groups * fx->splits, strideA_slice,
+                         strideW_bytes, (int64_t)M * N, terms == 22 ? amax_bits : nullptr, amax_rows, nullptr, stream, epi, fx);
 }
 
 extern "C" int sea_gemm_splitk_reduce(const float* partial, int splits, int M, int N, const float* bias, const float* addend,
@@ -645,7 +666,7 @@
 static int gemm_split_impl(const float* A, int64_t lda, const void* Wp, float* C, int64_t ldc, const float* bias, int relu, int M,
                            int N, int K, int terms, int batch, int64_t strideA, int64_t strideW_bytes, int64_t strideC,
                            const uint32_t* amax_bits, int amax_rows, uint32_t* out_amax, void* stream,
-                           const SeaGemmEpilogue* epi) {
+                           const SeaGemmEpilogue* epi, const SeaSplitKFixup* fx) {
   SEA_CHECK_ARG(A && Wp && C && M > 0 && N > 0 && K > 0 && (K % GS_BK) == 0 && batch > 0);
   SEA_CHECK_ARG(lda >= K && ldc >= N && (lda % 4) == 0 && (int64_t)M * lda < (1ll << 30));
   SEA_CHECK_ARG(((((uintptr_t)A) | ((uintptr_t)Wp)) & 15) == 0 && (((uintptr_t)C) & 3) == 0 && (strideA % 4) == 0 &&
@@ -685,6 +706,23 @@
   p.amax_mul = (epi && epi->a_amax_mul > 0.f) ? epi->a_amax_mul : 1.f;
   p.amax_mul_dev = epi ? epi->a_amax_mul_dev : nullptr;
   p.w_inv = terms == 22 ? (const float*)((const char*)Wp + (int64_t)(K / GS_BK) * 2 * gs_npad(N) * GS_BK * 2) : nullptr;
+  if (fx) {
+    p.fx_S = fx->splits;
+    p.fx_order = fx->slice_order != 0;
+    p.fx_relu = fx->relu;
+    p.fx_strideA_grp = fx->strideA_group;
+    p.fx_C = fx->C;
+    p.fx_ldc = fx->ldc;
+    p.fx_strideC = fx->strideC;
+    p.fx_bias = fx->bias;
+    p.fx_addend = fx->addend;
+    p.fx_ld_add = fx->ld_addend;
+    p.fx_stride_add = fx->stride_addend;
+    p.fx_out_amax = fx->out_amax;
+    p.fx_gelu_out = fx->gelu_out;
+    p.fx_gelu_grad_of = fx->gelu_grad_of;
+    p.fx_counters = fx->counters;
+  }
   const dim3 grid(p.per_xcd * 8), block(256);
   const bool shape16 = g_mfma_shape.load(std::memory_order_relaxed) == 16;
   const bool fused = p.addend || p.gelu_out || p.gelu_grad_of;
diff --git a/robust-segmentation_amd/csrc/gemm_split_big.hip b/robust-segmentation_amd/csrc/gemm_split_big.hip
--- a/robust-segmentation_amd/csrc/gemm_split_big.hip
+++ b/robust-segmentation_amd/csrc/gemm_split_big.hip
@@ -28,10 +28,8 @@
   const int64_t lda = p.lda, ldc = p.ldc;
   const int logical = (int)(blockIdx.x & 7) * p.per_xcd + (int)(blockIdx.x >> 3);
   if ((int)(blockIdx.x >> 3) >= p.per_xcd || logical >= p.total) return;
-  const int nb = logical % p.nblocks;
-  const int t2 = logical / p.nblocks;
-  const int mb = t2 % p.mblocks;
-  const int g = t2 / p.mblocks;
+  int g, mb, nb;
+  gemm_split_tile_of(p, logical, g, mb, nb);
   const int m0 = mb * BM, n0 = nb * BN;
   const float* const w_inv = F16 ? (const float*)((const char*)p.w_inv + (int64_t)g * p.strideW) : nullptr;
 
@@ -40,8 +38,8 @@
   const int r = lane & 31, h = lane >> 5;
   const int q = tid & 7, arow = tid >> 3;
 
-  const char* const Abase = (const char*)(p.A + (int64_t)g * p.strideA);
-  const char* const Tbase = HAS_T ? (const char*)(p.a_gelu_grad_of + (int64_t)g * p.strideA) : nullptr;
+  const char* const Abase = (const char*)(p.A + gemm_split_a_off(p, g));
+  const char* const Tbase = HAS_T ? (const char*)(p.a_gelu_grad_of + gemm_split_a_off(p, g)) : nullptr;
   const float* const bias = p.bias;
   const int nkb = K / GS_BK;
   const char* const Wbase = p.W + (int64_t)g * p.strideW + (int64_t)n0 * 64;
@@ -353,6 +351,7 @@
     }
     if (lane == 0 && omax > *(volatile uint32_t*)p.out_amax) atomicMax(p.out_amax, omax);
   }
+  if (p.fx_S > 1) gemm_split_fixup<BM, BN, NT>(p, g, mb, nb);
 }
 
 template <bool F16, int WM, int WN, int TN, int PRO, int DEPTH, int MI = 2, bool WDMA = false>
diff --git a/robust-segmentation_amd/csrc/gemm_split_pp.hip b/robust-segmentation_amd/csrc/gemm_split_pp.hip
--- a/robust-segmentation_amd/csrc/gemm_split_pp.hip
+++ b/robust-segmentation_amd/csrc/gemm_split_pp.hip
@@ -30,10 +30,8 @@
   const int64_t lda = p.lda, ldc = p.ldc;
   const int logical = (int)(blockIdx.x & 7) * p.per_xcd + (int)(blockIdx.x >> 3);
   if ((int)(blockIdx.x >> 3) >= p.per_xcd || logical >= p.total) return;
-  const int nb = logical % p.nblocks;
-  const int t2 = logical / p.nblocks;
-  const int mb = t2 % p.mblocks;
-  const int g = t2 / p.mblocks;
+  int g, mb, nb;
+  gemm_split_tile_of(p, logical, g, mb, nb);
   const int m0 = mb * GS_BM, n0 = nb * GS_BN;
   const float* const w_inv = F16 ? (const float*)((const char*)p.w_inv + (int64_t)g * p.strideW) : nullptr;
 
@@ -42,8 +40,8 @@
   const int r = lane & 31, h = lane >> 5;
   const int q = tid & 7, arow = tid >> 3;
 
-  const char* const Abase = (const char*)(p.A + (int64_t)g * p.strideA);
-  const char* const Tbase = HAS_T ? (const char*)(p.a_gelu_grad_of + (int64_t)g * p.strideA) : nullptr;
+  const char* const Abase = (const char*)(p.A + gemm_split_a_off(p, g));
+  const char* const Tbase = HAS_T ? (const char*)(p.a_gelu_grad_of + gemm_split_a_off(p, g)) : nullptr;
   const float* const bias = p.bias;
   const int relu = p.relu;
   const float* const addg = (EPI && p.addend) ? p.addend + (int64_t)g * p.stride_add : nullptr;
@@ -305,6 +303,7 @@
 #undef SEA_PIN
 
   gemm_split_store_tile<F16, EPI, KO>(p, acc, g, m0, n0, smem, row_inv, bv_c, wi_c);
+  if (p.fx_S > 1) gemm_split_fixup<GS_BM, GS_BN, 256>(p, g, mb, nb);
 }
 
 template <int TERMS, bool F16, bool EPI, int PRO, int DEPTH>
diff --git a/robust-segmentation_amd/semseg/_native.py b/robust-segmentation_amd/semseg/_native.py
--- a/robust-segmentation_amd/semseg/_native.py
+++ b/robust-segmentation_amd/semseg/_native.py
@@ -88,6 +88,7 @@
     "sea_wino_input_transform_amax": (_i, [_vp, _i64, _vp, _vp, _vp, _i64, _i, _i, _i, _i, _i, _vp, _vp]),
     "sea_gemm_split_fused": (_i, [_vp, _i64, _vp, _vp, _i64, _vp, _i, _i, _i, _i, _i, _i, _i64, _i64, _i64, _vp, _i, _vp, _vp, _vp]),
     "sea_gemm_splitk_reduce": (_i, [_vp, _i, _i, _i, _vp, _vp, _i64, _i, _vp, _i64, _vp, _vp]),
+    "sea_gemm_split_ksliced": (_i, [_vp, _i64, _vp, _vp, _i, _i, _i, _i, _i, _i64, _i64, _vp, _i, _vp, _vp, _vp]),
     "sea_gemm_split_packed_bytes": (_i64, [_i, _i, _i]),
     "sea_gemm_split_pack": (_i, [_vp, _i64, _i, _i, _i, _i, _vp, _vp]),
     "sea_gemm_split": (_i, [_vp, _i64, _vp, _vp, _i64, _vp, _i, _i, _i, _i, _i, _i, _i64, _i64, _i64, _vp]),
@@ -1046,6 +1047,11 @@
 
     def _slices_of(self, S):
         W, trans = self.src
+        if W.dim() == 3:
+            G = W.shape[0]
+            Ws = (W.view(G * S, self.K // S, self.N) if trans
+                  else W.view(G, self.N, S, self.K // S).permute(0, 2, 1, 3).reshape(G * S, self.N, self.K // S))
+            return gemm_split_pack(Ws, trans=trans, terms=self.terms)
         Ws = W.view(S, self.K // S, self.N) if trans else W.view(self.N, S, self.K // S).permute(1, 0, 2)
         return gemm_split_pack(Ws, trans=trans, terms=self.terms)
 
@@ -1081,7 +1087,7 @@
     for g in range(G):
         _check(L.sea_gemm_split_pack(_p(Wb[g]), Wb.stride(1), int(trans), N, K, terms, _p(out[g]), _stream()),
                "sea_gemm_split_pack")
-    return PackedWeight(out, N, K, terms, G, src=(W.detach(), trans) if (W.dim() == 2 and W.is_contiguous()) else None)
+    return PackedWeight(out, N, K, terms, G, src=(W.detach(), trans) if W.is_contiguous() else None)
 
 
 USE_MLP_FUSED = os.environ.get("SEA_MLP_FUSED", "1") != "0"
@@ -1229,11 +1235,15 @@
 
 KSPLIT = os.environ.get("SEA_GEMM_KSPLIT", "1") != "0"
 KSPLIT_BELOW, KSPLIT_TARGET, KSPLIT_MIN_KB = (int(v) for v in os.environ.get("SEA_GEMM_KSPLIT_PARAMS", "400,768,8").split(","))
+SPLITK_INKERNEL = os.environ.get("SEA_SPLITK_INKERNEL", "0") not in ("", "0")
+SPLITK_XCD = os.environ.get("SEA_SPLITK_XCD", "1") != "0" and os.environ.get("SEA_XCD_ORDER", "1") != "0"
+SPLITK_COUNTERS = 4096
 _ksplit_ws = {}
-
-
-def _ksplit(M, N, K):
-    blocks = -(-M // 128) * -(-N // 128)
+_ksplit_ctr = {}
+
+
+def _ksplit(M, N, K, G=1):
+    blocks = G * -(-M // 128) * -(-N // 128)
     nkb = K // 32
     if not KSPLIT or blocks >= KSPLIT_BELOW or N % 4:
         return 1
@@ -1251,8 +1261,31 @@
     return ws[:numel]
 
 
+def _ksplit_counters(device):
+    key = device.index if device.index is not None else torch.cuda.current_device()
+    ctr = _ksplit_ctr.get(key)
+    if ctr is None:
+        ctr = _ksplit_ctr[key] = torch.zeros(SPLITK_COUNTERS, dtype=torch.int32, device=device)
+    return ctr
+
+
+def ksplit_counters_reset(device):
+    ctr = _ksplit_ctr.get(device.index if device.index is not None else torch.cuda.current_device())
+    if ctr is not None:
+        ctr.zero_()
+
+
 def ksplit_workspace_pin(device):
-    return _ksplit_ws.get(device.index if device.index is not None else torch.cuda.current_device())
+    key = device.index if device.index is not None else torch.cuda.current_device()
+    ws, ctr = _ksplit_ws.get(key), _ksplit_ctr.get(key)
+    return None if (ws is None and ctr is None) else (ws, ctr)
+
+
+class _SplitKFixup(C.Structure):
+    _fields_ = [("splits", C.c_int), ("slice_order", C.c_int), ("relu", C.c_int), ("n_counters", C.c_int),
+                ("strideA_group", C.c_int64), ("C", C.c_void_p), ("ldc", C.c_int64), ("strideC", C.c_int64),
+                ("bias", C.c_void_p), ("addend", C.c_void_p), ("ld_addend", C.c_int64), ("stride_addend", C.c_int64),
+                ("out_amax", C.c_void_p), ("gelu_out", C.c_void_p), ("gelu_grad_of", C.c_void_p), ("counters", C.c_void_p)]
 
 
 class _GemmEpilogue(C.Structure):
@@ -1276,7 +1309,8 @@
 
 def gemm_split(A, Wp: PackedWeight, bias=None, relu: bool = False, out=None, amax=None, out_amax=None, addend=None,
                gelu_out=None, gelu_grad_of=None, amax_rows: int = 0, groups: int = 1, a_gelu_grad_of=None,
-               a_gelu: bool = False, a_relu_gate=None, row_amax: bool = False, amax_mul: float = 1.0):
+               a_gelu: bool = False, a_relu_gate=None, row_amax: bool = False, amax_mul: float = 1.0,
+               split_batched: bool = False):
     gate = a_relu_gate is not None
     if gate:
         if a_gelu_grad_of is not None:
@@ -1309,16 +1343,61 @@
     if a_gelu_grad_of is not None and (a_gelu_grad_of.shape != A.shape or a_gelu_grad_of.stride() != A.stride()
                                        or a_gelu_grad_of.dtype != torch.float32 or Wp.terms not in (1, 2, 22)):
         raise SeaNativeError("gemm_split: a_gelu_grad_of must be float32 with A's shape and strides (terms 1, 2 or 22)")
-    only_pro = gelu_out is None and gelu_grad_of is None
+    only_pro = (gelu_out is None and gelu_grad_of is None) or (
+        SPLITK_INKERNEL and addend is None and not relu and (bias is None or bias.data_ptr() % 16 == 0) and a_gelu_grad_of is None and not a_gelu and mul_dev is None
+        and amax_mul == 1.0 and all(t is None or (t.shape == out.shape and t.stride() == out.stride() and t.dtype == torch.float32
+                                                  and t.data_ptr() % 16 == 0) for t in (gelu_out, gelu_grad_of)))
     add_ok = addend is None or (addend.dim() == 2 and addend.shape == O3.shape[1:] and addend.stride(1) == 1
                                 and addend.stride(0) % 4 == 0 and addend.data_ptr() % 16 == 0 and addend.dtype == torch.float32)
-    if G == 1 and (not fused or (only_pro and add_ok)) and Wp.src is not None and O3.stride(1) % 4 == 0 and O3.data_ptr() % 16 == 0:
+    if G > 1 and split_batched and SPLITK_INKERNEL and not fused and Wp.src is not None and Wp.src[0].dim() == 3 \
+            and O3.stride(1) % 4 == 0 and O3.stride(0) % 4 == 0 and O3.data_ptr() % 16 == 0 \
+            and (bias is None or bias.data_ptr() % 16 == 0) and G * -(-M // 128) * -(-Wp.N // 128) <= SPLITK_COUNTERS:
+        S = _ksplit(M, Wp.N, K, G)
+        if S > 1:
+            if Wp.terms == 22 and amax is None:
+                amax, amax_rows = _amax_words(A3, M, K, G, sA, groups, row_amax)
+            part = _ksplit_workspace(A.device, G * S * M * Wp.N)
+            Ws = Wp.k_slices(S)
+            ctr = _ksplit_counters(A.device)
+            fx = _SplitKFixup(splits=S, slice_order=int(SPLITK_XCD), relu=int(relu), n_counters=ctr.numel(), strideA_group=sA,
+                              C=O3.data_ptr(), ldc=O3.stride(1), strideC=sC, bias=_p(bias), addend=None, ld_addend=0,
+                              stride_addend=0, out_amax=_p(out_amax) if Wp.terms == 22 else None, gelu_out=None,
+                              gelu_grad_of=None, counters=ctr.data_ptr())
+            _check(lib().sea_gemm_split_ksliced(_p(A3), A3.stride(1), _p(Ws.data), _p(part), M, Wp.N, K // S, Wp.terms, G,
+                                                K // S, Ws.stride, _p(amax) if Wp.terms == 22 else None, amax_rows, None,
+                                                C.addressof(fx), _stream()), "sea_gemm_split_ksliced")
+            return out
+    if G == 1 and (not fused or (only_pro and add_ok)) and Wp.src is not None and Wp.src[0].dim() == 2 \
+            and O3.stride(1) % 4 == 0 and O3.data_ptr() % 16 == 0:
         S = _ksplit(M, Wp.N, K)
         if S > 1:
             if Wp.terms == 22 and amax is None:
                 amax, amax_rows = _amax_words(A3, M, K, 1, 0, groups, row_amax)
             part = _ksplit_workspace(A.device, S * M * Wp.N).view(S, M, Wp.N)
             shape, strides = (S, M, K // S), (K // S, A3.stride(1), 1)
+            if SPLITK_INKERNEL and -(-M // 128) * -(-Wp.N // 128) <= SPLITK_COUNTERS and (bias is None or bias.data_ptr() % 16 == 0):
+                Ws = Wp.k_slices(S)
+                ctr = _ksplit_counters(A.device)
+                fx = _SplitKFixup(splits=S, slice_order=int(SPLITK_XCD), relu=int(relu), n_counters=ctr.numel(), strideA_group=0,
+                                  C=O3.data_ptr(), ldc=O3.stride(1), strideC=0, bias=_p(bias), addend=_p(addend),
+                                  ld_addend=addend.stride(0) if addend is not None else 0, stride_addend=0,
+                                  out_amax=_p(out_amax) if Wp.terms == 22 else None, gelu_out=_p(gelu_out),
+                                  gelu_grad_of=_p(gelu_grad_of), counters=ctr.data_ptr())
+                epi = None
+                if a_gelu_grad_of is not None or a_gelu or amax_mul != 1.0 or mul_dev is not None:
+                    epi = _GemmEpilogue()
+                    if a_gelu_grad_of is not None:
+                        epi.a_gelu_grad_of, epi.a_gate = a_gelu_grad_of.data_ptr(), int(gate)
+                    epi.a_gelu = int(bool(a_gelu))
+                    epi.a_amax_mul = amax_mul if amax_mul != 1.0 else 0.0
+                    epi.a_amax_mul_dev = mul_dev.data_ptr() if mul_dev is not None else None
+                _check(lib().sea_gemm_split_ksliced(_p(A3), A3.stride(1), _p(Ws.data), _p(part), M, Wp.N, K // S, Wp.terms, 1,
+                                                    K // S, Ws.stride, _p(amax) if Wp.terms == 22 else None, amax_rows,
+                                                    C.addressof(epi) if epi is not None else None, C.addressof(fx), _stream()),
+                       "sea_gemm_split_ksliced")
+                return out
+            if gelu_out is not None or gelu_grad_of is not None:
+                raise SeaNativeError("gemm_split: gelu_out / gelu_grad_of through split-K need the in-kernel fix-up")
             gemm_split(A3[0].as_strided(shape, strides), Wp.k_slices(S), out=part, amax=amax, amax_rows=amax_rows,
                        a_gelu_grad_of=None if (a_gelu_grad_of is None or gate) else a_gelu_grad_of.as_strided(shape, strides),
                        a_gelu=a_gelu, amax_mul=mul_dev if mul_dev is not None else amax_mul,
diff --git a/robust-segmentation_amd/semseg/attacker.py b/robust-segmentation_amd/semseg/attacker.py
--- a/robust-segmentation_amd/semseg/attacker.py
+++ b/robust-segmentation_amd/semseg/attacker.py
@@ -514,6 +514,7 @@
         print(f"[sea] HIP-graph capture of the attack step failed ({type(exc).__name__}: {str(exc).splitlines()[0][:160]}); "
               "continuing with the eager loop", file=sys.stderr)
         torch.cuda.synchronize()
+        N.ksplit_counters_reset(self.own.x.device)
 
     def _capture(self, i: int):
         o = self.own
diff --git a/robust-segmentation_amd/semseg/models/convnext_upernet.py b/robust-segmentation_amd/semseg/models/convnext_upernet.py
--- a/robust-segmentation_amd/semseg/models/convnext_upernet.py
+++ b/robust-segmentation_amd/semseg/models/convnext_upernet.py
@@ -339,6 +339,7 @@
 RELU_GATE_PROLOGUE = os.environ.get("SEA_RELU_GATE_PROLOGUE", "1") != "0"
 REDUCE_ADD = os.environ.get("SEA_REDUCE_ADD", "1") != "0"
 FUSE_PROLOGUE_MAX_NBLOCKS = int(os.environ.get("SEA_FUSE_PRO_NB", "3"))
+SPLITK_GELU = os.environ.get("SEA_SPLITK_GELU", "1") != "0"
 
 
 def _mlp_fusable(x, w1, b1, w2, b2):
@@ -381,6 +382,9 @@
             N.gemm_split(x2, _packed(w1, caches[0], "lin_fwd", False, terms), bias=b1, out=t, amax=a1, groups=nb)
             h = t
         elif fuse & 1:
+            h = torch.empty_like(t)
+            N.gemm_split(x2, _packed(w1, caches[0], "lin_fwd", False, terms), bias=b1, out=t, gelu_out=h, amax=a1, groups=nb)
+        elif SPLITK_GELU and N.SPLITK_INKERNEL and N._ksplit(x2.shape[0], w1.shape[0], w1.shape[1]) > 1:
             h = torch.empty_like(t)
             N.gemm_split(x2, _packed(w1, caches[0], "lin_fwd", False, terms), bias=b1, out=t, gelu_out=h, amax=a1, groups=nb)
         else:
@@ -429,6 +433,8 @@
             gx = N.gemm_split(N.gemm_split(g2, p2, gelu_grad_of=t, groups=nb, **rows), p1, groups=nb, **mul)
         elif ctx.fuse & 8 and terms in (1, 2, 22) and -(-ctx.w[0].shape[1] // 128) <= FUSE_PROLOGUE_MAX_NBLOCKS:
             gx = N.gemm_split(N.gemm_split(g2, p2, groups=nb, **rows), p1, a_gelu_grad_of=t, groups=nb, **mul)
+        elif SPLITK_GELU and N.SPLITK_INKERNEL and N._ksplit(g2.shape[0], ctx.w[1].shape[1], ctx.w[1].shape[0]) > 1:
+            gx = N.gemm_split(N.gemm_split(g2, p2, gelu_grad_of=t, groups=nb, **rows), p1, groups=nb, **mul)
         else:
             gx = N.gemm_split(torch.ops.aten.gelu_backward(N.gemm_split(g2, p2, groups=nb, **rows), t), p1, groups=nb, **mul)
         if ctx.kernel_fused and ctx.ln is not None:
diff --git a/robust-segmentation_amd/semseg/val.py b/robust-segmentation_amd/semseg/val.py
--- a/robust-segmentation_amd/semseg/val.py
+++ b/robust-segmentation_amd/semseg/val.py
@@ -167,6 +167,7 @@
                 except Exception as exc:
                     torch.cuda.set_stream(cur)
                     torch.cuda.synchronize()
+                    N.ksplit_counters_reset(X.device)
                     sl.failed = True
                     print(f"[sea] HIP-graph capture of the inner PGD failed ({type(exc).__name__}: "
                           f"{str(exc).splitlines()[0][:160]}); continuing with the eager loop", file=sys.stderr)
```
